# vasudeva-ram/Julia-NewtonRaphsonHANK

Measured on AMD Instinct MI355X. Metric: sequence-space JVPs/sec (household block: BackwardIteration+ForwardIteration+aggregation, Krusell-Smith T=300), higher is better.
Workload: dtype f64; 1 GPU; ks_2000x11_T300_N32; grid=2000x11, T=300, tangents_per_gpu=32, step=1 dual-sweep pass: primal + N tangents (hank_primal_jvp), parallelism=tangent-sharded x1

## Files before the change

### julia-newtonraphsonhank_amd/csrc/hank_hip.hip

```cpp
#include "hank_kernels.h"
#include "hank_xsweep.h"
#include "hank_jacobian.h"
#include "hank_wide.h"
#include "hank_hetx.h"
#include "hank_adjoint.h"
#include "hank_boundary.h"
#include "hank_ssdiff_launch.h"
#include "../../include/hank_hip.h"

#include <cstdarg>
#include <cstdio>
#include <cstdlib>
#include <cstring>
#include <initializer_list>
#include <list>
#include <mutex>
#include <new>
#include <vector>

using namespace hank;

struct FreeDevice { void operator()(void *p) const { (void)hipFree(p); } };
struct FreeGraphExec { void operator()(hipGraphExec_t g) const { (void)hipGraphExecDestroy(g); } };
template <typename H, typename Release>
// ... 702 lines not shown
    HIPC(ctx, hipMemsetAsync(X.sync, 0, sizeof(XSync) * ((size_t)2 + 2 * XPASS_MAX), ctx->stream));
    HIPC(ctx, X.st_s.alloc(2 * XG * G));
    HIPC(ctx, X.st_ds.alloc(2 * XG * G * X.dmax));
    const size_t GM = (size_t)c.n_e * X.Sact * 64;
    HIPC(ctx, X.st_D.alloc(2 * XG * std::max(GV, GM)));
    HIPC(ctx, X.st_dD.alloc(2 * XG * GM * xslots(X.dmax + 1).SP));
    HIPC(ctx, X.Dvirt.alloc(P * c.n_e * 64));
    HIPC(ctx, X.D0own.alloc(P * c.n_e));
    HIPC(ctx, X.aggpart.alloc(2 * P * (size_t)X.Sact));
    HIPC(ctx, X.rho.alloc(P));
    HIPC(ctx, X.srcB.alloc(P * X.Sact));
    HIPC(ctx, X.srcF.alloc(P * X.Sact));
    HIPC(ctx, X.unitsF.alloc(P * X.Sact * XUCAP));
    HIPC(ctx, X.unit_overflow.alloc(1));
    HIPC(ctx, hipMemsetAsync(X.unit_overflow, 0, sizeof(int), ctx->stream));
    if (const char *ng = getenv("HANK_XNEIGH")) X.neigh = atoi(ng) != 0;
    if (const char *uc = getenv("HANK_XUCAP")) X.ucap = std::min(XUCAP, std::max(1, atoi(uc)));
    {
        double ms = 20.0;
        if (const char *wm = getenv("HANK_XWAIT_MS")) ms = atof(wm);
        const unsigned long long ticks = (unsigned long long)(std::max(ms, 0.01) * 1e5);
        HIPC(ctx, hipMemcpyToSymbol(HIP_SYMBOL(hank::g_xwait_ticks), &ticks, sizeof(ticks)));
    }
    if (const char *sv = getenv("HANK_XSYNCWAVE")) X.syncwave = atoi(sv) != 0;
    X.lds_max = (int)prop.sharedMemPerBlock;
    if (const char *xf = getenv("HANK_XFAULT")) {
        X.fault = strncmp(xf, "placement", 9) == 0 ? XERR_PLACEMENT : (strncmp(xf, "timeout", 7) == 0 ? XERR_TIMEOUT : (strncmp(xf, "stall", 5) == 0 ? 3 : 0));
        const char *w = strchr(xf, ':');
        X.fault_where = !w ? 7 : (strcmp(w, ":primal") == 0 ? 1 : (strcmp(w, ":tangent") == 0 ? 2 : (strcmp(w, ":fixedpoint") == 0 ? 4 : 7)));
    }
    HIPC(ctx, hipMemsetAsync(X.Dvirt, 0, sizeof(double) * P * c.n_e * 64, ctx->stream));
    X.ready = true;
    return HANK_OK;
}

static int x_build_tan(hank_ctx *ctx, XTan &w) {
    XWork &X = ctx->xw;
    const Consts &c = ctx->c;
    const size_t P = c.P, G = c.G;
    const int N = w.N;
    size_t off = 0;
    for (int n0 = 0; n0 < N; n0 += XG * X.dmax) {
        XPass ps;
        ps.n0 = n0; ps.N = std::min(N - n0, XG * X.dmax);
        ps.D = 1; while (XG * ps.D < ps.N) ps.D *= 2;
        ps.groups = (ps.N + ps.D - 1) / ps.D;
        ps.dpol_off = off;
        off += P * ps.groups * G * ps.D;
        w.passes.push_back(ps);
    }
    if ((int)w.passes.size() > XPASS_MAX) return fail(ctx, HANK_ERR_BAD_ARG, "N=%d needs %d passes, at most %d per call", N, (int)w.passes.size(), XPASS_MAX);
    HIPC(ctx, w.dxhh.alloc((size_t)c.n_hh * P * N));
    HIPC(ctx, w.dxr.alloc(P * N)); HIPC(ctx, w.dxw.alloc(P * N)); HIPC(ctx, w.dxt.alloc(P * N));
    HIPC(ctx, w.dpol.alloc(off));
    const size_t W = (size_t)XG * X.dmax, nb = (size_t)X.Sact;
    HIPC(ctx, w.daggpart.alloc(2 * P * nb * W));
    HIPC(ctx, hipMemsetAsync(w.daggpart, 0, sizeof(double) * 2 * P * nb * W, ctx->stream));
    HIPC(ctx, w.dagg_pass.alloc(2 * P * W));
    HIPC(ctx, w.dagg_cm.alloc(2 * P * N));
    return HANK_OK;
}
static int x_ensure_tan(hank_ctx *ctx, int N, XTan **out) {
    const int nmax = 8 * ctx->xw.dmax * XPASS_MAX;
    if (N > nmax) return fail(ctx, HANK_ERR_BAD_ARG, "N=%d exceeds %d directions per call", N, nmax);
    return tan_cache_get(ctx, ctx->xw.tans, N, [ctx](XTan &w) { return x_build_tan(ctx, w); }, out);
}

static dim3 x_block(const XWork &X, const Consts &c) {
    const bool fits = 64 * (c.n_e + 1) <= X.maxt && X.syncwave;
    return dim3(fits ? 64 * (c.n_e + 1) : 64 * c.n_e);
}

template <typename F>
static void x_by_maxt(const XWork &X, F launch) { if (X.maxt == 768) launch(std::integral_constant<int, 768>()); else launch(std::integral_constant<int, 1024>()); }
#define XL(...) hipLaunchKernelGGL((__VA_ARGS__), dim3(X.grid), x_block(X, c), lds, sec.stream(), a)
static bool x_has_dual_back(const XWork &X) { return X.maxt == 768; }
static void x_launch_dual_back(XSection &sec, const XWork &X, const Consts &c, int D, const XDualBackArgs &a) {
    const size_t lds = x_lds_dual_back(c, D);
    if (!x_has_dual_back(X)) return;
    if (D == 1) XL(k_xdual_back<1, 768>);
    else if (D == 2) XL(k_xdual_back<2, 768>);
    else XL(k_xdual_back<4, 768>);
}
static void x_launch_fwd(XSection &sec, const XWork &X, const Consts &c, int D, bool val, const XSweepFwdArgs &a) {
    const size_t lds = x_lds_fwd(c, D, val || D == 0);
    x_by_maxt(X, [&](auto mt) {
        constexpr int MT = decltype(mt)::value;
        if (D == 0) XL(k_xfwd<0, true, MT>);
        else if (D == 1) { if (val) XL(k_xfwd<1, true, MT>); else XL(k_xfwd<1, false, MT>); }
        else if (D == 2) { if (val) XL(k_xfwd<2, true, MT>); else XL(k_xfwd<2, false, MT>); }
        else if (D == 4) { if constexpr (MT == 768) { if (val) XL(k_xfwd<4, true, MT>); else XL(k_xfwd<4, false, MT>); } }
    });
}
static void x_launch_primal_back(XSection &sec, const XWork &X, const Consts &c, const XBackArgs &a) { const size_t lds = x_lds_primal_back(c); x_by_maxt(X, [&](auto mt) { XL(k_xprimal_back<decltype(mt)::value>); }); }
static void x_launch_tan_back(XSection &sec, const XWork &X, const Consts &c, int D, const XTanBackArgs &a) {
    const size_t lds = x_lds_tan_back(c, D);
    x_by_maxt(X, [&](auto mt) {
        constexpr int MT = decltype(mt)::value;
        if (D == 1) XL(k_xtan_back<1, MT>);
        else if (D == 2) XL(k_xtan_back<2, MT>);
        else if (D == 4) { if constexpr (MT == 768) XL(k_xtan_back<4, MT>); }
    });
}
static void x_ensure_rng(XSection &sec) {
    hank_ctx *ctx = sec.ctx;
    XWork &X = ctx->xw;
    if (X.rng_valid) return;
    hipLaunchKernelGGL(k_xunits_fwd, dim3((unsigned)ctx->c.P, (unsigned)X.Sact), dim3(256), 0, sec.stream(), ctx->c, ctx->R, X.Sact, X.srcF, X.unitsF, X.unit_overflow, X.ucap);
    X.rng_valid = true;
}

static int ensure_seg(hank_ctx *ctx) {
    if (ctx->seg_valid) return HANK_OK;
    hipLaunchKernelGGL(k_seg_build, dim3((unsigned)(ctx->c.P * ctx->c.n_e)), dim3(256), 0, ctx->stream, ctx->c, ctx->R, ctx->c.P * ctx->c.n_e);
    HIPC(ctx, hipGetLastError());
    ctx->seg_valid = true;
    return HANK_OK;
}
static int ensure_lwg(hank_ctx *ctx) {
    if (ctx->lwg_valid) return HANK_OK;
    const XWork &X = ctx->xw;
    hipLaunchKernelGGL(k_xlwg_build, dim3((unsigned)(ctx->c.P * ctx->c.n_e)), dim3(256), 0, ctx->stream, ctx->c, ctx->R, X.Dvirt, X.D0own, X.Sact);
    HIPC(ctx, hipGetLastError());
    ctx->lwg_valid = true;
    ctx->lwg_builds++;
    return HANK_OK;
}
static int x_sync_reset(XSection &sec, XSync *base, int count, int where) {
    hank_ctx *ctx = sec.ctx;
    HIPC(ctx, hipMemsetAsync(base, 0, sizeof(XSync) * (size_t)count, sec.stream()));
    if (ctx->xw.fault && ctx->xw.fault != 3 && (ctx->xw.fault_where & where)) hipLaunchKernelGGL(k_xpoison, dim3(1), dim3(64), 0, sec.stream(), base, count, (unsigned)ctx->xw.fault);
    return HANK_OK;
}

static void x_rho(XSection &sec) {
    hank_ctx *ctx = sec.ctx;
    hipLaunchKernelGGL(k_xrho, dim3((unsigned)((ctx->c.P + 255) / 256)), dim3(256), 0, sec.stream(), ctx->d_xhh, ctx->c.n_hh, ctx->c.P, ctx->xw.rho);
}
static void x_tan_in(XSection &sec, XTan *w) {
    const Consts &c = sec.ctx->c;
    hipLaunchKernelGGL(k_tan_in, dim3((unsigned)(((size_t)c.P * w->N + 255) / 256)), dim3(256), 0, sec.stream(), w->dxhh, c.n_hh, c.P, w->N, w->dxr, w->dxw, w->dxt);
}
static int x_tan_front(XSection &sec, XTan *w) {
    hank_ctx *ctx = sec.ctx; XWork &X = ctx->xw;
    const int rc = x_sync_reset(sec, X.sync + 2, 2 * (int)w->passes.size(), 2); if (rc) return rc;
    x_tan_in(sec, w);
    x_rho(sec);
    if (!X.src_valid) {
        hipLaunchKernelGGL(k_xsrc_back, dim3((unsigned)ctx->c.P, X.Sact), dim3(256), 0, sec.stream(), ctx->c, ctx->R, X.Sact, X.srcB);
        X.src_valid = true;
    }
    return HANK_OK;
}
static int x_back(XSection &sec, XTan *dual = nullptr) {
    hank_ctx *ctx = sec.ctx; XWork &X = ctx->xw;
    const Consts &c = ctx->c;
    XBackArgs ab{};
    ab.c = c; ab.ss_value = ctx->d_ss_value; ab.xhh = ctx->d_xhh; ab.rho = X.rho; ab.sy = X.sync; ab.st_s = X.st_s;
    ab.err = ctx->d_err; ab.R = ctx->R;
    HIPC(ctx, ctx->spans.begin(PRIMAL_BACK, sec.stream()));
    if (dual) {
        const XPass &ps = dual->passes[0];
        XDualBackArgs db{};
        db.p = ab; db.dxr = dual->dxr; db.dxw = dual->dxw; db.dxt = dual->dxt; db.Ntot = dual->N; db.n0 = ps.n0; db.N = ps.N;
        db.st_ds = X.st_ds; db.dpol = dual->dpol + ps.dpol_off; db.groups = ps.groups;
        x_launch_dual_back(sec, X, c, ps.D, db);
    } else x_launch_primal_back(sec, X, c, ab);
    HIPC(ctx, ctx->spans.end(PRIMAL_BACK, sec.stream(), 1));
    return HANK_OK;
}
static void x_lottery(XSection &sec, bool seg) {
    hank_ctx *ctx = sec.ctx;
    const Consts &c = ctx->c;
    hipLaunchKernelGGL(k_lottery, dim3((unsigned)(c.P * c.n_e)), dim3(256), sizeof(int) * (2 * (size_t)c.n_a + 2), sec.stream(), c, ctx->R, c.P * c.n_e, ctx->d_err, seg ? 1 : 0, 1);
}
static int x_tan_back(XSection &sec, XTan *w) {
    hank_ctx *ctx = sec.ctx; XWork &X = ctx->xw;
    const int np = (int)w->passes.size();
    XTanBackArgs ab{};
    ab.c = ctx->c; ab.R = ctx->R; ab.rho = X.rho; ab.xhh = ctx->d_xhh; ab.dxr = w->dxr; ab.dxw = w->dxw; ab.dxt = w->dxt; ab.Ntot = w->N; ab.st_ds = X.st_ds;
    ab.src = X.neigh ? X.srcB.get() : nullptr;
    ab.stall = X.fault == 3 ? 1 : 0;
    HIPC(ctx, ctx->spans.begin(TAN_BACK, sec.stream()));
    for (int p = 0; p < np; p++) {
        const XPass &ps = w->passes[p];
        ab.n0 = ps.n0; ab.N = ps.N; ab.groups = ps.groups; ab.sy = X.sync + 2 + 2 * p; ab.dpol = w->dpol + ps.dpol_off;
        x_launch_tan_back(sec, X, ctx->c, ps.D, ab);
    }
    HIPC(ctx, ctx->spans.end(TAN_BACK, sec.stream(), np));
    return HANK_OK;
}
static void x_value_epilogue(XSection &sec) {
    hank_ctx *ctx = sec.ctx; const XWork &X = ctx->xw;
    const Consts &c = ctx->c;
    const size_t P = c.P;
    hipStream_t s = sec.stream();
    hipLaunchKernelGGL(k_reduce_parts, dim3((unsigned)P, 1), dim3(256), 0, s, X.aggpart, X.Sact, 2, ctx->d_agg_rm);
    hipLaunchKernelGGL(k_tan_out, dim3((unsigned)((2 * P + 255) / 256)), dim3(256), 0, s, ctx->d_agg_rm, (int)P, 2, ctx->d_agg);
    hipLaunchKernelGGL(k_xfix_D, dim3((unsigned)((P * c.n_e + 255) / 256)), dim3(256), 0, s, c, ctx->R.Dseq, X.Dvirt, X.Sact, X.D0own);
}
static XSweepFwdArgs x_fwd_args(const hank_ctx *ctx, bool val) {
    const XWork &X = ctx->xw;
    XSweepFwdArgs fa{};
    fa.c = ctx->c; fa.R = ctx->R; fa.src = X.srcF; fa.units = X.unitsF; fa.overflow = X.unit_overflow; fa.all_members = X.neigh ? 0 : 1;
    if (val) { fa.D0 = ctx->d_ss_D; fa.Dvirt = X.Dvirt; fa.aggpart = X.aggpart; }
    return fa;
}
static int x_fwd_value(XSection &sec) {
    hank_ctx *ctx = sec.ctx; XWork &X = ctx->xw;
    XSweepFwdArgs fa = x_fwd_args(ctx, true);
    fa.sy = X.sync + 1; fa.st = X.st_D; fa.groups = 1;
    HIPC(ctx, ctx->spans.begin(PRIMAL_FWD, sec.stream()));
    x_launch_fwd(sec, X, ctx->c, 0, true, fa);
    HIPC(ctx, ctx->spans.end(PRIMAL_FWD, sec.stream(), 1));
    x_value_epilogue(sec);
    return HANK_OK;
}
static int x_tan_fwd(XSection &sec, XTan *w, int p, bool val) {
    hank_ctx *ctx = sec.ctx; XWork &X = ctx->xw;
    const XPass &ps = w->passes[p];
    if (!val) { const int rc = ensure_lwg(ctx); if (rc) return rc; }
    XSweepFwdArgs fa = x_fwd_args(ctx, val);
    fa.sy = X.sync + 2 + 2 * p + 1; fa.st = X.st_dD; fa.daggpart = w->daggpart; fa.groups = ps.groups; fa.dpol = w->dpol + ps.dpol_off;
    x_launch_fwd(sec, X, ctx->c, ps.D, val, fa);
    return HANK_OK;
}
static void x_tan_reduce(XSection &sec, XTan *w, int p) {
    hank_ctx *ctx = sec.ctx;
    const size_t P = ctx->c.P;
    const XPass &ps = w->passes[p];
    const int W = XG * ps.D;
    hipStream_t s = sec.stream();
    hipLaunchKernelGGL(k_reduce_parts, dim3((unsigned)P, (2 * W + 63) / 64), dim3(256), 0, s, w->daggpart, ctx->xw.Sact, 2 * W, w->dagg_pass);
    hipLaunchKernelGGL(k_xout, dim3((unsigned)((P * ps.N + 255) / 256)), dim3(256), 0, s, w->dagg_pass, (int)P, 2 * W, 0, ps.n0, ps.N, w->dagg_cm);
    hipLaunchKernelGGL(k_xout, dim3((unsigned)((P * ps.N + 255) / 256)), dim3(256), 0, s, w->dagg_pass, (int)P, 2 * W, W, ps.n0, ps.N, w->dagg_cm + P * (size_t)w->N);
}
static int x_tan_fwd_from(XSection &sec, XTan *w, int first) {
    hank_ctx *ctx = sec.ctx;
    const int np = (int)w->passes.size();
    for (int p = first; p < np; p++) {
        const int rc = x_tan_fwd(sec, w, p, false); if (rc) return rc;
        if (p == np - 1) HIPC(ctx, ctx->spans.end(TAN_FWD, sec.stream(), np));
        x_tan_reduce(sec, w, p);
    }
    return HANK_OK;
}
static void x_dual_epilogue(XSection &sec, XTan *w, double *d_agg_out, double *d_dagg_out) {
    hank_ctx *ctx = sec.ctx; const XWork &X = ctx->xw;
    const Consts &c = ctx->c;
    const XPass &ps = w->passes[0];
    const int W = XG * ps.D, per = 2 * W + 2 + c.n_e;
    hipLaunchKernelGGL(k_xdual_epilogue, dim3((unsigned)(((size_t)c.P * per + 255) / 256)), dim3(256), 0, sec.stream(), c, X.aggpart, w->daggpart, X.Sact, W, ps.n0, ps.N, w->N,
                       ctx->d_agg_rm, ctx->d_agg, w->dagg_pass, w->dagg_cm, ctx->R.Dseq, X.Dvirt, X.D0own, d_agg_out, d_dagg_out);
}

static int x_status(hank_ctx *ctx, const char *what, const XSync *fetched) {
    XWork &X = ctx->xw;
    std::vector<XSync> own;
    if (!fetched) {
        if (!X.ready || X.last_blocks == 0) return HANK_OK;
        int uo = 0;
        HIPC(ctx, hipMemcpy(&uo, X.unit_overflow, sizeof(int), hipMemcpyDeviceToHost));
        if (uo) {
            HIPC(ctx, hipMemsetAsync(X.unit_overflow, 0, sizeof(int), ctx->stream));
            return fail(ctx, HANK_ERR_SWEEP, "persistent forward sweep: a member's walk over its sources needs more than %d work units (a savings policy this flat is served by the per-period launches)", XUCAP);
        }
        own.resize((size_t)X.last_blocks);
        HIPC(ctx, hipMemcpy(own.data(), X.sync, sizeof(XSync) * own.size(), hipMemcpyDeviceToHost));
    }
    const XSync *h = fetched ? fetched : own.data();
    for (size_t k = 0; k < (fetched ? 1 : own.size()); k++)
        if (h[k].status[0] != 0) {
            if (what) return fail(ctx, HANK_ERR_SWEEP, "persistent %s: %s on XCD %u", what, h[k].status[0] == XERR_PLACEMENT ? "the group is short of members" : "a wait timed out", h[k].status[1]);
            char waited[64] = "";
            if (h[k].status[0] == XERR_TIMEOUT) snprintf(waited, sizeof(waited), " after %.1f ms", h[k].status[2] / 1000.0);
            return fail(ctx, HANK_ERR_SWEEP, "persistent %s sweep %zu (0 = primal, then one per tangent pass): %s%s on XCD %u (workgroups per XCD: %u %u %u %u %u %u %u %u)",
                        (k & 1) ? "forward" : "backward", k / 2, h[k].status[0] == XERR_PLACEMENT ? "a group is short of members" : "a wait timed out", waited,
                        h[k].status[1], h[k].ticket[0][0], h[k].ticket[1][0], h[k].ticket[2][0], h[k].ticket[3][0], h[k].ticket[4][0],
                        h[k].ticket[5][0], h[k].ticket[6][0], h[k].ticket[7][0]);
        }
    return HANK_OK;
}

#define HANK_WIDE_NE_LIST(X) X(2) X(3) X(4) X(5) X(7) X(11)
static bool w_ne_instantiated(int ne) {
#define X(NEV) if (ne == NEV) return true;
    HANK_WIDE_NE_LIST(X)
#undef X
    return false;
}
struct WGeom { int R, maxt, kreg_b, kreg_f; };
static WGeom w_geom(const hank_ctx *ctx) { return ctx->wide_r == 2 ? WGeom{2, 1024, 16, 7} : WGeom{4, 512, 16, 16}; }
static int w_threads(const hank_ctx *ctx) { const WGeom g = w_geom(ctx); return std::max(64, ((ctx->c.n_a + g.R - 1) / g.R + 63) / 64 * 64); }
static size_t w_lds(const hank_ctx *ctx) { const WGeom g = w_geom(ctx); return std::max(wide_lds_back(ctx->c, g.kreg_b), wide_lds_fwd(ctx->c, g.kreg_f)); }
static bool w_supported(const hank_ctx *ctx) {
    const Consts &c = ctx->c;
    return w_ne_instantiated(c.n_e) && c.n_a <= WIDE_CS && w_lds(ctx) <= ctx->lds_max &&
           ctx->rec_bytes < 0x7fffffffull && (size_t)c.G * sizeof(double) < 0x7fffffffull;
}
static bool use_wide(const hank_ctx *ctx, int N) {
    if (ctx->wide_mode == 2) return true;
    if (ctx->wide_mode != 1) return false;
    const int rounds = (N + ctx->num_cus - 1) / ctx->num_cus;
    return (long long)N * 256 >= (long long)rounds * ctx->wide_min * ctx->num_cus;
}

template <int NE, int R, int MAXT, int KB, int KF>
static int w_launch_geom(XSection &sec, bool fwd, int N, const WideArgs &a) {
    hank_ctx *ctx = sec.ctx;
    const Consts &c = ctx->c;
    WMat<NE> M;
    for (int k = 0; k < NE; k++)
        for (int e = 0; e < NE; e++) M.m[k * NE + e] = fwd ? ctx->h_Pi[k + NE * e] : ctx->h_Pi[e + NE * k];
    for (int e = 0; e < NE; e++) M.z[e] = ctx->h_z[e];
    const dim3 grd((unsigned)N), blk((unsigned)w_threads(ctx));
    if (fwd) {
        const size_t lds = wide_lds_fwd(c, KF);
        HIPC(ctx, hipFuncSetAttribute(reinterpret_cast<const void *>(&k_wide_fwd<NE, R, MAXT, KF>), hipFuncAttributeMaxDynamicSharedMemorySize, (int)lds));
        hipLaunchKernelGGL((k_wide_fwd<NE, R, MAXT, KF>), grd, blk, lds, sec.stream(), a, M);
    } else {
        const size_t lds = wide_lds_back(c, KB);
        if (c.diet) {
            HIPC(ctx, hipFuncSetAttribute(reinterpret_cast<const void *>(&k_wide_back<NE, R, MAXT, true, KB>), hipFuncAttributeMaxDynamicSharedMemorySize, (int)lds));
            hipLaunchKernelGGL((k_wide_back<NE, R, MAXT, true, KB>), grd, blk, lds, sec.stream(), a, M);
        } else {
            HIPC(ctx, hipFuncSetAttribute(reinterpret_cast<const void *>(&k_wide_back<NE, R, MAXT, false, KB>), hipFuncAttributeMaxDynamicSharedMemorySize, (int)lds));
            hipLaunchKernelGGL((k_wide_back<NE, R, MAXT, false, KB>), grd, blk, lds, sec.stream(), a, M);
        }
    }
    return HANK_OK;
}
static int w_launch(XSection &sec, bool fwd, int N, const WideArgs &a) {
    hank_ctx *ctx = sec.ctx;
#define X(NEV) if (ctx->c.n_e == NEV) return ctx->wide_r == 2 ? w_launch_geom<NEV, 2, 1024, 16, 7>(sec, fwd, N, a) : w_launch_geom<NEV, 4, 512, 16, 16>(sec, fwd, N, a);
    HANK_WIDE_NE_LIST(X)
#undef X
    return fail(ctx, HANK_ERR_BAD_ARG, "on-chip wide sweeps: n_e=%d is not instantiated", ctx->c.n_e);
}

static int w_ensure_tan(hank_ctx *ctx, int N, bool staging, WTan **out) {
    const size_t P = ctx->c.P, G = ctx->c.G;
    const int rc = tan_cache_get(ctx, ctx->wtans, N, [=](WTan &w) -> int {
        HIPC(ctx, w.dpol.alloc(P * (size_t)N * G + 2));
        HIPC(ctx, w.dagg_cm.alloc(2 * P * (size_t)N));
        return HANK_OK;
    }, out);
    if (rc) return rc;
    if (staging && !(*out)->dxhh) HIPC(ctx, (*out)->dxhh.alloc((size_t)ctx->c.n_hh * P * N));
    return HANK_OK;
}

static int w_run_tangent(hank_ctx *ctx, WTan *w, const double *d_dxhh) {
    const Consts &c = ctx->c;
    XSection sec(ctx);
    HIPC(ctx, sec.opened());
    hipStream_t s = sec.stream();
    if (!ctx->d_ibw) HIPC(ctx, ctx->d_ibw.alloc((size_t)c.P * c.G + 4));
    WideArgs a{};
    a.c = c; a.R = ctx->R; a.xhh = ctx->d_xhh; a.dxhh = d_dxhh; a.Ntot = w->N; a.n0 = 0; a.dpol = w->dpol; a.dagg = w->dagg_cm;
    a.rec = ctx->rec_slab;
    auto off = [&](const void *p) { return (unsigned)((const char *)p - ctx->rec_slab); };
    const Record &R = ctx->R;
    a.o_s = off(R.s); a.o_kc = off(R.kc); a.o_u = off(R.u); a.o_v = off(R.v); a.ibw = ctx->d_ibw;
    a.nrank = std::max(1, std::min(ctx->num_cus / 8, w->N / 8));
    a.o_lwg = off(R.lwg); a.o_start = off(R.start); a.o_D = off(R.Dseq); a.o_pol = off(R.pol);
    if (!ctx->wprep_valid) {
        const size_t npt = (size_t)c.P * c.G;
        hipLaunchKernelGGL(k_wide_prep, dim3((unsigned)((npt + 255) / 256)), dim3(256), 0, s, R.ib, R.A, R.B, npt, ctx->d_ibw);
        ctx->wprep_valid = true;
    }
    HIPC(ctx, ctx->spans.begin(TAN_BACK, s));
    int rc = w_launch(sec, false, w->N, a);
    if (rc) return rc;
    HIPC(ctx, ctx->spans.end(TAN_BACK, s, 1));
    HIPC(ctx, join_side(ctx));
    rc = ensure_lwg(ctx);
// ... 258 lines not shown
    HIPC(ctx, hipEventRecord(ctx->ev_fork, ctx->stream));
    HIPC(ctx, hipStreamWaitEvent(ctx->side_stream, ctx->ev_fork, 0));
    HIPC(ctx, ctx->spans.begin(PRIMAL_FWD, ctx->side_stream));
    HIPC(ctx, hipGraphLaunch(ctx->g_pfwd, ctx->side_stream));
    HIPC(ctx, ctx->spans.end(PRIMAL_FWD, ctx->side_stream, ctx->c.P + 1));
    HIPC(ctx, copy_agg(ctx, d_agg_out, hipMemcpyDeviceToDevice, ctx->side_stream));
    HIPC(ctx, hipEventRecord(ctx->ev_side, ctx->side_stream));
    ctx->side_pending = true;
    ctx->spans.invalidate({DUAL_BACK, DUAL_FWD});
    record_rewritten(ctx, true, true);
    return HANK_OK;
}

static int x_primal(hank_ctx *ctx, const double *xhh, hipMemcpyKind kind, double *d_agg_out) {
    int rc = x_setup(ctx); if (rc) return rc;
    HIPC(ctx, hipMemcpyAsync(ctx->d_xhh, xhh, sizeof(double) * ctx->c.n_hh * ctx->c.P, kind, ctx->stream));
    XSection sec(ctx);
    HIPC(ctx, sec.opened());
    rc = x_sync_reset(sec, ctx->xw.sync, 2, 1); if (rc) return rc;
    zero_err(ctx, sec.stream());
    x_rho(sec);
    rc = x_back(sec); if (rc) return rc;
    x_lottery(sec, true);
    record_rewritten(ctx, true, HANK_XPRIMAL_LWG_IN_SWEEP);
    x_ensure_rng(sec);
    rc = x_fwd_value(sec); if (rc) return rc;
    HIPC(ctx, hipGetLastError());
    HIPC(ctx, sec.close());
    ctx->stats[SWEEP_LAUNCHES] += 2;
    ctx->xw.last_blocks = 2;
    ctx->spans.invalidate({TAN_BACK, TAN_FWD, DUAL_BACK, DUAL_FWD});
    HIPC(ctx, copy_agg(ctx, d_agg_out, hipMemcpyDeviceToDevice, ctx->stream));
    return HANK_OK;
}
static int x_jvp(hank_ctx *ctx, const double *dxhh, hipMemcpyKind kind, int N, double *d_dagg_out) {
    int rc = x_setup(ctx); if (rc) return rc;
    XTan *w = nullptr;
    rc = x_ensure_tan(ctx, N, &w); if (rc) return rc;
    const int np = (int)w->passes.size();
    HIPC(ctx, hipMemcpyAsync(w->dxhh, dxhh, sizeof(double) * ctx->c.n_hh * ctx->c.P * N, kind, ctx->stream));
    XSection sec(ctx);
    HIPC(ctx, sec.opened());
    rc = x_tan_front(sec, w); if (rc) return rc;
    x_ensure_rng(sec);
    rc = x_tan_back(sec, w); if (rc) return rc;
    HIPC(ctx, ctx->spans.begin(TAN_FWD, sec.stream()));
    rc = x_tan_fwd_from(sec, w, 0); if (rc) return rc;
    HIPC(ctx, hipGetLastError());
    HIPC(ctx, sec.close());
    ctx->stats[SWEEP_LAUNCHES] += 2 * np;
    ctx->xw.last_blocks = 2 + 2 * np;
    ctx->spans.invalidate({DUAL_BACK, DUAL_FWD});
    batch_ran(ctx, 1, w, N, w->dagg_cm, w->dpol, &w->passes);
    HIPC(ctx, copy_dagg(ctx, d_dagg_out, w->dagg_cm, N, hipMemcpyDeviceToDevice));
    return HANK_OK;
}
static void x_dual_ran(hank_ctx *ctx, XTan *w, int launches) {
    ctx->stats[SWEEP_LAUNCHES] += launches;
    ctx->xw.last_blocks = 2 + 2 * (int)w->passes.size();
    ctx->spans.absent(PRIMAL_FWD, 1);
    ctx->spans.invalidate({DUAL_BACK, DUAL_FWD});
    batch_ran(ctx, 1, w, w->N, w->dagg_cm, w->dpol, &w->passes);
}
static int x_dual_two(hank_ctx *ctx, XTan *w, const double *xhh, const double *dxhh, hipMemcpyKind kind, double *d_agg_out, double *d_dagg_out) {
    const size_t nP = (size_t)ctx->c.n_hh * ctx->c.P;
    const int np = (int)w->passes.size();
    XSection sec(ctx);
    HIPC(ctx, sec.opened());
    HIPC(ctx, hipMemcpyAsync(w->dxhh, dxhh, sizeof(double) * nP * w->N, kind, sec.stream()));
    HIPC(ctx, hipMemcpyAsync(ctx->d_xhh, xhh, sizeof(double) * nP, kind, sec.stream()));
    int rc = x_sync_reset(sec, ctx->xw.sync, 2, 1); if (rc) return rc;
    zero_err(ctx, sec.stream());
    x_rho(sec);
    rc = x_back(sec); if (rc) return rc;
    x_lottery(sec, true);
    record_rewritten(ctx, true, false);
    x_ensure_rng(sec);
    rc = x_tan_front(sec, w);
    if (!rc) rc = x_tan_back(sec, w);
    if (rc) return rc;
    HIPC(ctx, ctx->spans.begin(TAN_FWD, sec.stream()));
    rc = x_tan_fwd(sec, w, 0, true); if (rc) return rc;
    if (np == 1) {
        HIPC(ctx, ctx->spans.end(TAN_FWD, sec.stream(), 1));
        x_dual_epilogue(sec, w, d_agg_out, d_dagg_out);
    } else {
        x_value_epilogue(sec);
        x_tan_reduce(sec, w, 0);
        rc = x_tan_fwd_from(sec, w, 1); if (rc) return rc;
    }
    HIPC(ctx, hipGetLastError());
    HIPC(ctx, sec.close());
    x_dual_ran(ctx, w, 1 + 2 * np);
    if (np > 1) {
        HIPC(ctx, copy_agg(ctx, d_agg_out, hipMemcpyDeviceToDevice, ctx->stream));
        HIPC(ctx, copy_dagg(ctx, d_dagg_out, w->dagg_cm, w->N, hipMemcpyDeviceToDevice));
    }
    return HANK_OK;
}
static int x_dual_fused(hank_ctx *ctx, XTan *w, const double *xhh, const double *dxhh, hipMemcpyKind kind, bool prologue, double *d_agg_out, double *d_dagg_out) {
    XWork &X = ctx->xw;
    const size_t nP = (size_t)ctx->c.n_hh * ctx->c.P;
    XSection sec(ctx);
    HIPC(ctx, sec.opened());
    if (prologue) {
        hipLaunchKernelGGL(k_xdual_prologue, dim3(64), dim3(256), 0, sec.stream(), xhh, ctx->d_xhh, dxhh, w->dxhh, ctx->c.n_hh, ctx->c.P, w->N, X.rho, w->dxr, w->dxw, w->dxt,
                           reinterpret_cast<xv4u *>(X.sync.get()), sizeof(XSync) * 4 / sizeof(xv4u), ctx->d_err);
    } else {
        HIPC(ctx, hipMemcpyAsync(w->dxhh, dxhh, sizeof(double) * nP * w->N, kind, sec.stream()));
        HIPC(ctx, hipMemcpyAsync(ctx->d_xhh, xhh, sizeof(double) * nP, kind, sec.stream()));
        int rc = x_sync_reset(sec, X.sync, 2, 1);
        if (!rc) rc = x_sync_reset(sec, X.sync + 2, 2, 2);
        if (rc) return rc;
        zero_err(ctx, sec.stream());
        x_rho(sec);
        x_tan_in(sec, w);
    }
    int rc = x_back(sec, w); if (rc) return rc;
    x_lottery(sec, false);
    record_rewritten(ctx, false, false);
    x_ensure_rng(sec);
    HIPC(ctx, ctx->spans.begin(TAN_BACK, sec.stream()));
    HIPC(ctx, ctx->spans.end(TAN_BACK, sec.stream(), 1));
    HIPC(ctx, ctx->spans.begin(TAN_FWD, sec.stream()));
    rc = x_tan_fwd(sec, w, 0, true); if (rc) return rc;
    HIPC(ctx, ctx->spans.end(TAN_FWD, sec.stream(), 1));
    x_dual_epilogue(sec, w, d_agg_out, d_dagg_out);
    HIPC(ctx, hipGetLastError());
    HIPC(ctx, sec.close());
    x_dual_ran(ctx, w, 2);
    return HANK_OK;
}
static bool x_dual_back_fits(const hank_ctx *ctx, int D);
static int x_dual(hank_ctx *ctx, const double *xhh, const double *dxhh, hipMemcpyKind kind, int N, double *d_agg_out, double *d_dagg_out) {
    int rc = x_setup(ctx); if (rc) return rc;
    XTan *w = nullptr;
    rc = x_ensure_tan(ctx, N, &w); if (rc) return rc;
    if (w->passes.size() != 1 || !x_dual_back_fits(ctx, w->passes[0].D)) return x_dual_two(ctx, w, xhh, dxhh, kind, d_agg_out, d_dagg_out);
    return x_dual_fused(ctx, w, xhh, dxhh, kind, kind == hipMemcpyDeviceToDevice && !ctx->xw.fault, d_agg_out, d_dagg_out);
}
static bool use_x_primal(const hank_ctx *ctx) { return ctx->schedule >= 1; }
static bool x_tan_fits(const hank_ctx *ctx, int N) {
    const XWork &X = ctx->xw;
    int D = 1;
    while (XG * D < N && D < X.dmax) D *= 2;
    return std::max(x_lds_tan_back(ctx->c, D), x_lds_fwd(ctx->c, D, true)) <= (size_t)X.lds_max;
}
static bool use_x_jvp(const hank_ctx *ctx, int N) { return (ctx->schedule == 1 || (ctx->schedule == 2 && N <= ctx->xjvp_max)) && x_tan_fits(ctx, N); }
static bool x_dual_back_fits(const hank_ctx *ctx, int D) {
    const XWork &X = ctx->xw;
    return ctx->xdual_back && x_has_dual_back(X) && 64 * (ctx->c.n_e + 1) <= X.maxt && x_lds_dual_back(ctx->c, D) <= (size_t)X.lds_max;
}
static bool use_x_fused(const hank_ctx *ctx, int N) {
    if (ctx->schedule < 1 || !x_tan_fits(ctx, N)) return false;
    if (ctx->schedule == 1) return true;
    return N <= XG * ctx->xw.dmax && x_dual_back_fits(ctx, ctx->xw.dmax);
}

static int check_rates(hank_ctx *ctx, const double *xhh) {
    for (int t = 0; t < ctx->c.P; t++)
        if (!(1.0 + xhh[ctx->c.n_hh * t] > 0.0)) return fail(ctx, HANK_ERR_DOMAIN, "1 + r must be positive (period %zu)", (size_t)t + 1);
    return HANK_OK;
}
static int enqueue_primal(hank_ctx *ctx, const double *xhh, hipMemcpyKind kind, double *d_agg_out) {
    if (use_x_primal(ctx)) return x_primal(ctx, xhh, kind, d_agg_out);
    HIPC(ctx, hipMemcpyAsync(ctx->d_xhh, xhh, sizeof(double) * ctx->c.n_hh * ctx->c.P, kind, ctx->stream));
    return run_primal(ctx, d_agg_out);
}

int hank_primal_dev(hank_ctx *ctx, const double *d_xhh, double *d_agg_out) {
    ENTER(ctx);
    if (!ctx || !d_xhh) return fail(ctx, HANK_ERR_BAD_ARG, "null pointer");
    if (!ctx->boundary_set) return fail(ctx, HANK_ERR_NOT_READY, "hank_set_boundary must be called first");
    note_primal_x(ctx, nullptr);
    ctx->stats[PRIMAL_SWEEPS]++;
    return enqueue_primal(ctx, d_xhh, hipMemcpyDeviceToDevice, d_agg_out);
}

int hank_check(hank_ctx *ctx) {
    ENTER(ctx);
    if (!ctx) return HANK_ERR_BAD_ARG;
    bool moved = false;
    return fallback_decision(ctx, device_verdict(ctx, THE_RECORD), &moved);
}

int hank_primal(hank_ctx *ctx, const double *xhh, double *agg_out) {
    ENTER(ctx);
    if (!ctx || !xhh) return fail(ctx, HANK_ERR_BAD_ARG, "null pointer");
    if (!ctx->boundary_set) return fail(ctx, HANK_ERR_NOT_READY, "hank_set_boundary must be called first");
    { const int rrc = check_rates(ctx, xhh); if (rrc) return rrc; }
    note_primal_x(ctx, nullptr);
    const int rc = run_settled(ctx, [&] { return enqueue_primal(ctx, xhh, hipMemcpyHostToDevice, nullptr); });
    if (rc) return rc;
    if (agg_out) {
        HIPC(ctx, copy_agg(ctx, agg_out, hipMemcpyDeviceToHost, ctx->stream));
        HIPC(ctx, hipStreamSynchronize(ctx->stream));
    }
    note_primal_x(ctx, xhh);
    ctx->stats[PRIMAL_SWEEPS]++;
    ctx->errmsg[0] = 0;
    return HANK_OK;
}

static int run_jvp(hank_ctx *ctx, TanWork &w, bool bnd, bool zm, int NX) {
    const int grc = ensure_tan_graphs(ctx, w, bnd, NX);
    if (grc) return grc;
    HIPC(ctx, ctx->spans.begin(TAN_BACK, ctx->stream));
    HIPC(ctx, hipGraphLaunch(w.tan_back(bnd), ctx->stream));
    HIPC(ctx, ctx->spans.end(TAN_BACK, ctx->stream, ctx->c.P + (bnd ? 4 : 2)));
    HIPC(ctx, join_side(ctx));
    { const int src = ensure_seg(ctx); if (src) return src; }
    { const int src = ensure_lwg(ctx); if (src) return src; }
    HIPC(ctx, ctx->spans.begin(TAN_FWD, ctx->stream));
    HIPC(ctx, hipGraphLaunch(w.tan_fwd(bnd, NX), ctx->stream));
    HIPC(ctx, ctx->spans.end(TAN_FWD, ctx->stream, ctx->c.P + (bnd ? 5 : 3) + (NX > 0 ? 1 : 0)));
    if (bnd) batch_ran_boundary(ctx, &w, w.N, w.dagg_cm, w.dpol, zm ? w.bnd_zm.get() : nullptr);
    else batch_ran(ctx, 0, &w, w.N, w.dagg_cm, w.dpol);
    return HANK_OK;
}

struct TanReq {
    int n_het;
    const double *dxhh, *dvalue_end, *dD_init;
    hipMemcpyKind kind;
    bool seeded;
};
static int ensure_bnd_bufs(hank_ctx *ctx, TanWork &w);
static int ensure_hx_record(hank_ctx *ctx);

static int enqueue_tan_launch(hank_ctx *ctx, const TanReq &q, int N, TanWork **out) {
    const Consts &c = ctx->c;
    const size_t P = c.P, GN = (size_t)c.G * N;
    const int NX = q.n_het > 2 ? q.n_het - 2 : 0, SX = hx_count(ctx);
    TanWork *w = nullptr;
    int rc = ensure_tanwork(ctx, N, &w);
    if (rc) return rc;
    if (q.seeded && (rc = ensure_bnd_bufs(ctx, *w)) != HANK_OK) return rc;
    if (q.n_het > 0 && !w->het_out) HIPC(ctx, w->het_out.alloc(P * het_max(ctx) * N));
    if (NX > 0) {
        HIPC(ctx, join_side(ctx));
        rc = ensure_hx_record(ctx);
        if (rc) return rc;
        if (!w->hx_T) {
            HIPC(ctx, w->hx_parts.alloc(P * (size_t)w->nbf * SX * N));
            HIPC(ctx, w->hx_T.alloc((size_t)N * P * SX));
        }
    }
    const struct { double *dst; const double *src; size_t count; } in[3] = {{w->dxhh, q.dxhh, c.n_hh * P * N}, {w->bnd_dV, q.dvalue_end, GN}, {w->bnd_dD, q.dD_init, GN}};
    for (int k = 0; k < (q.seeded ? 3 : 1); k++) {
        if (in[k].src) HIPC(ctx, hipMemcpyAsync(in[k].dst, in[k].src, sizeof(double) * in[k].count, q.kind, ctx->stream));
        else HIPC(ctx, hipMemsetAsync(in[k].dst, 0, sizeof(double) * in[k].count, ctx->stream));
    }
    rc = run_jvp(ctx, *w, q.seeded, q.dD_init != nullptr, NX);
    if (rc) return rc;
    *out = w;
    return HANK_OK;
}
static int enqueue_tan_raw(hank_ctx *ctx, const TanReq &q, int N, double *d_dagg_out) {
    TanWork *w = nullptr;
    const int rc = enqueue_tan_launch(ctx, q, N, &w);
    if (rc) return rc;
    HIPC(ctx, copy_dagg(ctx, d_dagg_out, w->dagg_cm, N, hipMemcpyDeviceToDevice));
    return HANK_OK;
}
static int tan_host_tail(hank_ctx *ctx, double *out, const double *d_src, size_t count) {
    HIPC(ctx, hipMemcpyAsync(out, d_src, sizeof(double) * count, hipMemcpyDeviceToHost, ctx->stream));
    HIPC(ctx, hipStreamSynchronize(ctx->stream));
    ctx->errmsg[0] = 0;
    return HANK_OK;
}
static int tan_seed_args(hank_ctx *ctx, const char *who, bool het, const TanReq &q, int N, const void *out, bool need_out) {
    if (!ctx || (!q.dxhh && !q.dvalue_end && !q.dD_init) || (need_out && !out) || N < 1)
        return fail(ctx, HANK_ERR_BAD_ARG, "%s: bad argument (N=%d; at least one of dxhh, dvalue_end, dD_init must be given)", who, N);
    const int rc = het ? het_count_ok(ctx, who, q.n_het, true) : HANK_OK;
    if (rc) return rc;
    if (!ctx->primal_done) return fail(ctx, HANK_ERR_NOT_READY, "hank_primal must be called before %s", who);
    return HANK_OK;
}

static int enqueue_jvp(hank_ctx *ctx, const double *dxhh, hipMemcpyKind kind, int N, double *d_dagg_out) {
    if (use_wide(ctx, N)) return w_jvp(ctx, dxhh, kind, N, d_dagg_out);
    if (use_x_jvp(ctx, N)) return x_jvp(ctx, dxhh, kind, N, d_dagg_out);
    return enqueue_tan_raw(ctx, TanReq{0, dxhh, nullptr, nullptr, kind, false}, N, d_dagg_out);
}

int hank_jvp_dev(hank_ctx *ctx, const double *d_dxhh, int32_t N, double *d_dagg_out) {
    ENTER(ctx);
    if (!ctx || !d_dxhh || N < 1) return fail(ctx, HANK_ERR_BAD_ARG, "bad argument (N=%d)", N);
    if (!ctx->primal_done) return fail(ctx, HANK_ERR_NOT_READY, "hank_primal must be called before hank_jvp");
    return enqueue_jvp(ctx, d_dxhh, hipMemcpyDeviceToDevice, N, d_dagg_out);
}

int hank_jvp(hank_ctx *ctx, const double *dxhh, int32_t N, double *dagg_out) {
    ENTER(ctx);
    if (!ctx || !dxhh || !dagg_out || N < 1) return fail(ctx, HANK_ERR_BAD_ARG, "bad argument (N=%d)", N);
    if (!ctx->primal_done) return fail(ctx, HANK_ERR_NOT_READY, "hank_primal must be called before hank_jvp");
    int rc = enqueue_jvp(ctx, dxhh, hipMemcpyHostToDevice, N, nullptr);
    if (rc) return rc;
    if (ctx->batch.family == 2) rc = device_verdict(ctx, THE_RECORD);
    else if (ctx->batch.family == 1) {
        bool rerun = false;
        rc = settle(ctx, &rerun);
        if (rerun) {
            rc = run_primal(ctx, nullptr);
            if (!rc) rc = device_verdict(ctx, THE_RECORD);
            if (!rc) rc = enqueue_jvp(ctx, dxhh, hipMemcpyHostToDevice, N, nullptr);
        }
// ... 1306 lines not shown
```

### julia-newtonraphsonhank_amd/csrc/hank_kernels.h

```cpp
#pragma once
#include <hip/hip_runtime.h>
#include <stdint.h>

namespace hank {

constexpr int RBP = 32;

struct Consts {
    int n_a, n_e, G, P;
    int n_hh;
    int diet;
    double beta, gamma, bc;
    const double *a, *z, *Pi;
};

struct Record {
    double *s, *kc, *A, *B, *u, *v, *pol, *lw, *ig, *Dseq;
    int *ib, *lo, *start, *clo;
    int4 *seg;
    double2 *lwg;
};

enum { ERR_KNOTS = 3, ERR_DOMAIN = 4, ERR_NONMONO = 6 };

__device__ inline void set_err(int *err, int code, int t, int e, int j) {
    if (atomicCAS(&err[0], 0, code) == 0) {
        err[1] = t;
        err[2] = e;
        err[3] = j;
    }
}

__device__ inline bool pow_domain_error(double v, double y) { return (v < 0.0) && (y != floor(y)); }

#ifndef HANK_IEEE_DIV
#define HANK_IEEE_DIV 0
#endif
__device__ __forceinline__ double fast_rcp(double x) {
#if HANK_IEEE_DIV
    return 1.0 / x;
#else
    double r = __builtin_amdgcn_rcp(x);
    r = __builtin_fma(__builtin_fma(-x, r, 1.0), r, r);
    r = __builtin_fma(__builtin_fma(-x, r, 1.0), r, r);
    return r;
#endif
}
__device__ __forceinline__ double fast_rsqrt(double x) {
#if HANK_IEEE_DIV
    return 1.0 / sqrt(x);
#else
    double y = __builtin_amdgcn_rsq(x);
    y = __builtin_fma(y * 0.5, __builtin_fma(-(x * y), y, 1.0), y);
    y = __builtin_fma(y * 0.5, __builtin_fma(-(x * y), y, 1.0), y);
    return y;
#endif
}
__device__ __forceinline__ double fast_sqrt(double x) {
#if HANK_IEEE_DIV
    return sqrt(x);
#else
    const double y = fast_rsqrt(x), g = x * y;
    return __builtin_fma(y * 0.5, __builtin_fma(-g, g, x), g);
#endif
}

__device__ inline double pow_crra(double x, double y) {
    if (y == -0.5) return fast_rsqrt(x);
    if (y == -2.0) return fast_rcp(x * x);
    if (y == -1.0) return fast_rcp(x);
    return pow(x, y);
}

__device__ inline double wave_sum(double x) {
#pragma unroll
    for (int off = 32; off > 0; off >>= 1) x += __shfl_down(x, off, 64);
    return x;
}
__device__ inline double block_sum(double x, double *red, int nthreads) {
    const int lane = threadIdx.x & 63, wv = threadIdx.x >> 6;
    const int nw = (nthreads + 63) >> 6;
    x = wave_sum(x);
    __syncthreads();
    if (lane == 0) red[wv] = x;
    __syncthreads();
    double r = 0.0;
    if (threadIdx.x == 0)
        for (int k = 0; k < nw; k++) r += red[k];
    return r;
}

#ifndef HANK_RAW_BARRIER
#define HANK_RAW_BARRIER 1
#endif
__device__ __forceinline__ void lds_barrier() {
#if HANK_RAW_BARRIER
    asm volatile("s_waitcnt lgkmcnt(0)\n\ts_barrier" ::: "memory");
#else
    __syncthreads();
#endif
}

#ifndef HANK_ST_DPOL
#define HANK_ST_DPOL 1
#endif
#ifndef HANK_ST_STATE
#define HANK_ST_STATE 1
#endif
#ifndef HANK_ST_REC
#define HANK_ST_REC 0
#endif
template <int MODE>
__device__ __forceinline__ void st_mode(double *p, double x) {
    if (MODE == 1) __hip_atomic_store(reinterpret_cast<unsigned long long *>(p), (unsigned long long)__double_as_longlong(x), __ATOMIC_RELAXED, __HIP_MEMORY_SCOPE_AGENT);
    else if (MODE == 2) __builtin_nontemporal_store(x, p);
    else *p = x;
}
template <int MODE>
__device__ __forceinline__ void st_mode_i(int *p, int x) {
    if (MODE == 1) __hip_atomic_store(p, x, __ATOMIC_RELAXED, __HIP_MEMORY_SCOPE_AGENT);
    else if (MODE == 2) __builtin_nontemporal_store(x, p);
    else *p = x;
}

__device__ __forceinline__ double mix_mul(double p, double v) { return p * v; }
__device__ __forceinline__ double2 mix_mul(double p, double2 v) { return make_double2(p * v.x, p * v.y); }
__device__ __forceinline__ double mix_add(double a, double b) { return a + b; }
__device__ __forceinline__ double2 mix_add(double2 a, double2 b) { return make_double2(a.x + b.x, a.y + b.y); }
template <typename T>
__device__ __forceinline__ T mix_sum(T acc, const T *V, int vs, const double *P, int ps, int k0, int n) {
    int k = k0;
    for (; k + 3 < n; k += 4) {
        const T v0 = V[k * vs], v1 = V[(k + 1) * vs], v2 = V[(k + 2) * vs], v3 = V[(k + 3) * vs];
        const double p0 = P[k * ps], p1 = P[(k + 1) * ps], p2 = P[(k + 2) * ps], p3 = P[(k + 3) * ps];
        acc = mix_add(acc, mix_mul(p0, v0));
        acc = mix_add(acc, mix_mul(p1, v1));
        acc = mix_add(acc, mix_mul(p2, v2));
        acc = mix_add(acc, mix_mul(p3, v3));
    }
    if (k + 1 < n) {
        const T v0 = V[k * vs], v1 = V[(k + 1) * vs];
        const double p0 = P[k * ps], p1 = P[(k + 1) * ps];
        acc = mix_add(acc, mix_mul(p0, v0));
        acc = mix_add(acc, mix_mul(p1, v1));
        k += 2;
    }
    if (k < n) acc = mix_add(acc, mix_mul(P[k * ps], V[k * vs]));
    return acc;
}

__device__ __forceinline__ double diet_kc(const Consts &c, double s, double rho, double opr, double wz_tr, double xa) {
    const double cm = (s * opr + wz_tr) - xa;
    const double k = rho * (c.beta * (-1.0 / c.gamma));
    return c.gamma == 2.0 ? k * (cm * cm * cm) : k * (cm * cm);
}
__device__ __forceinline__ double diet_v(const Consts &c, double u, double opr) {
    return c.gamma == 2.0 ? opr * (-2.0 * (u * fast_sqrt(u))) : opr * (-(u * u));
}

__device__ __forceinline__ double hh_tr(const Consts &c, const double *xhh, int t) { return c.n_hh > 2 ? xhh[c.n_hh * t + 2] : 0.0; }

__device__ inline void egm_X(const Consts &c, const double *Vsh, const double *Pish, int row, int a,
                             int e, double r, double w, double tr, double *s_out, double *kc_out, int *err,
                             int t) {
    const double E = mix_sum(Vsh[row] * Pish[e], Vsh + row, RBP, Pish + e, c.n_e, 1, c.n_e);
    const double bE = E * c.beta;
    const double ex = -1.0 / c.gamma;
    if (pow_domain_error(bE, ex)) set_err(err, ERR_DOMAIN, t, e, a);
    const double cm = pow_crra(bE, ex);
    const double rho = 1.0 / (1.0 + r);
    const double s1 = rho * ((cm - (w * c.z[e] + tr)) + c.a[a]);
    st_mode<HANK_ST_REC>(s_out, s1);
    st_mode<HANK_ST_REC>(kc_out, c.diet ? diet_kc(c, s1, rho, 1.0 + r, w * c.z[e] + tr, c.a[a]) : rho * (c.beta * ex * (cm / bE)));
}

struct YOut {
    double g, A, B, u, v, V;
    int ib;
};
enum { Y_INSIDE = 0, Y_BELOW = 1, Y_ABOVE = 2 };
struct YFront {
    int where, i;
    double si, sj;
    bool slow;
    bool bad;
};
template <typename KNOTS> struct YFrontOf { static constexpr bool value = false; };
template <typename KNOTS> struct YColumnZOf { static constexpr bool value = false; };
constexpr int Y_WAIT_VMCNT0 = 0x0F70;

template <bool ZREG>
__device__ __forceinline__ YOut egm_Y_finish(const Consts &c, int a, int e, double r, double w, double tr, int *err, int t,
                                             double x, double g, double A, double B, int i, double ze) {
    YOut o;
    const double bc = c.bc;
    if ((bc > g) || ((int)signbit(bc) < (int)signbit(g))) {
        A = 0.0;
        B = 0.0;
    }
    g = (g > bc) ? g : ((bc > g) ? bc : (signbit(g) ? bc : g));
    const double opr = 1.0 + r;
    const double cg = (opr * x + (w * (ZREG ? ze : c.z[e]) + tr)) - g;
    if (pow_domain_error(cg, -c.gamma)) set_err(err, ERR_DOMAIN, t, e, a);
    const double u = pow_crra(cg, -c.gamma);
    o.g = g;
    o.A = A;
    o.B = B;
    o.ib = i;
    o.u = u;
    o.v = c.diet ? diet_v(c, u, opr) : opr * ((-c.gamma) * (u / cg));
    o.V = opr * u;
    return o;
}

template <typename KNOTS>
__device__ inline YOut egm_Y(const Consts &c, const KNOTS sc, int a, int e, double r, double w, double tr,
                             int *err, int t, int guess) {
    constexpr bool FRONT = YFrontOf<KNOTS>::value;
    const int n = c.n_a;
    const double x = c.a[a];
    double s0, sN, si, sj;
    int where, i;
    bool slow, slow_wave;
    if constexpr (FRONT) {
        const YFront f = sc.front(x, guess);
        where = f.where; i = f.i; si = f.si; sj = f.sj;
        slow = f.slow;
        slow_wave = __any(f.slow || f.bad) != 0;
        if (slow_wave) {
            if (f.bad) set_err(err, ERR_KNOTS, t, e, a);
        }
    } else {
        const double sa = sc[a];
        if (a > 0 ? !(sa > sc[a - 1]) : !(sa == sa)) set_err(err, ERR_KNOTS, t, e, a);
        s0 = sc[0]; sN = sc[n - 1];
    }
    double g, A = 0.0, B = 0.0;
    if (FRONT ? where == Y_BELOW : x < s0) {
        g = c.a[0];
        i = 0;
    } else if (FRONT ? where == Y_ABOVE : x > sN) {
        g = c.a[n - 1];
        i = n - 2;
    } else {
        if (FRONT ? slow_wave : true) {
            if (FRONT ? slow : true) {
                int lo = -1, hi = n;
                bool have = false;
                double vlo = 0.0, vhi = 0.0;
                if (guess >= 0) {
                    const int p = guess < n - 1 ? guess : n - 2;
                    const int pm = p > 0 ? p - 1 : 0, pp = p + 2 < n ? p + 2 : n - 1;
                    const double sm = sc[pm], sp = sc[p], sp1 = sc[p + 1], sp2 = sc[pp];
                    if (sp <= x && x < sp1) {
                        lo = p; hi = p + 1; have = true; vlo = sp; vhi = sp1;
                    } else if (p + 2 < n && sp1 <= x && x < sp2) {
                        lo = p + 1; hi = p + 2; have = true; vlo = sp1; vhi = sp2;
                    } else if (p > 0 && sm <= x && x < sp) {
                        lo = p - 1; hi = p; have = true; vlo = sm; vhi = sp;
                    } else if (sp1 <= x) {
                        lo = p + 1;
                        for (int step = 1;; step <<= 1) {
                            const int q = lo + step;
                            if (q >= n) break;
                            if (sc[q] <= x) lo = q; else { hi = q; break; }
                        }
                    } else {
                        hi = p;
                        for (int step = 1;; step <<= 1) {
                            const int q = hi - step;
                            if (q < 0) break;
                            if (sc[q] <= x) { lo = q; break; } else hi = q;
                        }
                    }
                }
                while (hi - lo > 1) {
// ... 861 lines not shown
```

### julia-newtonraphsonhank_amd/csrc/hank_wide.h

```cpp
#pragma once
#include "hank_xsweep.h"

namespace hank {

constexpr int WIDE_CS = 2048;
constexpr int wide_kl(int ne, int kreg) { return ne > kreg ? ne - kreg : 0; }
template <int NE> struct WMat { double m[NE * NE]; double z[NE]; };

__device__ __forceinline__ double wide_uniform(double v) {
    return __hiloint2double(__builtin_amdgcn_readfirstlane(__double2hiint(v)), __builtin_amdgcn_readfirstlane(__double2loint(v)));
}
__device__ __forceinline__ void wide_pin(double &v) { asm volatile("" : "+v"(v)); }
__device__ __forceinline__ int wide_opaque_zero(int t, int q) { return __builtin_amdgcn_readfirstlane((t >> (27 + (q & 3))) & 1); }

template <int NE, int R, int KR, int LSTRIDE>
__device__ __forceinline__ void wide_mix(double (&x)[R][KR], double *lst, const double *m, int zero) {
#pragma clang fp contract(fast)
    constexpr int KL = NE - KR;
    double y[R][NE], cf[2][NE], xl[2][R];
    int off = zero;
#pragma unroll
    for (int e = 0; e < NE; e++) cf[0][e] = m[off + e];
#pragma unroll
    for (int k = 0; k < NE; k++) {
        if (k + 1 < NE) {
            if (k == 0) asm volatile("" : "+s"(off) : "v"(x[0][0]));
            else asm volatile("" : "+s"(off) : "v"(y[R - 1][NE - 1]));
#pragma unroll
            for (int e = 0; e < NE; e++) cf[(k + 1) & 1][e] = m[off + (k + 1) * NE + e];
            if (k + 1 >= KR) {
#pragma unroll
                for (int q = 0; q < R; q++) xl[(k + 1) & 1][q] = lst[((k + 1 - KR) * R + q) * LSTRIDE];
            }
        }
        if (k == 0 && KR == 0) {
#pragma unroll
            for (int q = 0; q < R; q++) xl[0][q] = lst[q * LSTRIDE];
        }
#pragma unroll
        for (int q = 0; q < R; q++) {
            const double xk = k < KR ? x[q][k < KR ? k : 0] : xl[k & 1][q];
#pragma unroll
            for (int e = 0; e < NE; e++) { y[q][e] = k == 0 ? cf[0][e] * xk : y[q][e] + cf[k & 1][e] * xk; asm volatile("" : "+v"(y[q][e])); }
        }
        __builtin_amdgcn_sched_barrier(0);
    }
#pragma unroll
    for (int q = 0; q < R; q++) {
#pragma unroll
        for (int e = 0; e < KR; e++) { x[q][e] = y[q][e]; asm volatile("" : "+v"(x[q][e])); }
#pragma unroll
        for (int k = 0; k < KL; k++) lst[(k * R + q) * LSTRIDE] = y[q][KR + k];
    }
    __builtin_amdgcn_sched_barrier(0);
}

typedef unsigned int wv2u __attribute__((ext_vector_type(2)));
typedef unsigned int wv4u __attribute__((ext_vector_type(4)));
__device__ __forceinline__ __amdgpu_buffer_rsrc_t wide_rsrc(const void *p) {
    return __builtin_amdgcn_make_buffer_rsrc(const_cast<void *>(p), 0, 0x7fffffff, 0x00020000);
}
__device__ __forceinline__ double wide_ld64(__amdgpu_buffer_rsrc_t rs, int vo, int so) {
    const wv2u q = __builtin_amdgcn_raw_buffer_load_b64(rs, vo, so, 0);
    return __hiloint2double((int)q.y, (int)q.x);
}
__device__ __forceinline__ wv2u wide_ld2i(__amdgpu_buffer_rsrc_t rs, int vo, int so) { return __builtin_amdgcn_raw_buffer_load_b64(rs, vo, so, 0); }
template <int AUX>
__device__ __forceinline__ void wide_ld2d(__amdgpu_buffer_rsrc_t rs, int vo, int so, double &a, double &b) {
    const wv4u q = __builtin_amdgcn_raw_buffer_load_b128(rs, vo, so, AUX);
    a = __hiloint2double((int)q.y, (int)q.x); b = __hiloint2double((int)q.w, (int)q.z);
}
__device__ __forceinline__ wv4u wide_ld128(__amdgpu_buffer_rsrc_t rs, int vo, int so) { return __builtin_amdgcn_raw_buffer_load_b128(rs, vo, so, 0); }
__device__ __forceinline__ void wide_st2d_nt(double a, double b, __amdgpu_buffer_rsrc_t rs, int vo, int so) {
    wv4u q;
    q.x = (unsigned)__double2loint(a); q.y = (unsigned)__double2hiint(a); q.z = (unsigned)__double2loint(b); q.w = (unsigned)__double2hiint(b);
    __builtin_amdgcn_raw_buffer_store_b128(q, rs, vo, so, 2);
}
__device__ __forceinline__ void wide_st64_nt(double v, __amdgpu_buffer_rsrc_t rs, int vo, int so) {
    wv2u q;
    q.x = (unsigned)__double2loint(v); q.y = (unsigned)__double2hiint(v);
    __builtin_amdgcn_raw_buffer_store_b64(q, rs, vo, so, 2);
}

#ifdef HANK_WIDE_TIMING_L2
#define WIDE_TPER(t) ((t) & 1)
#else
#define WIDE_TPER(t) (t)
#endif
#ifdef HANK_XSTAMP
__device__ unsigned long long g_wstamps[2][4][64];
#define WSTAMP(sw, per, i)                                                                                          \
    do {                                                                                                            \
        if (blockIdx.x == 0 && threadIdx.x == 0 && (per) >= 100 && (per) < 104) g_wstamps[sw][(per) - 100][i] = __builtin_amdgcn_s_memtime(); \
    } while (0)
#else
#define WSTAMP(sw, per, i) do {} while (0)
#endif

struct WideArgs {
    Consts c;
    Record R;
    const double *xhh;
    const double *dxhh;
    int Ntot, n0;
    double *dpol;
    double *dagg;
    const void *rec;
    unsigned o_s, o_kc, o_u, o_v, o_lwg, o_start, o_D, o_pol;
    const int *ibw;
    int nrank;
};

static inline size_t wide_lds_back(const Consts &c, int kreg) {
    return sizeof(double) * (4 * (size_t)WIDE_CS + (size_t)WIDE_CS + 8 * (size_t)c.P + (size_t)wide_kl(c.n_e, kreg) * WIDE_CS);
}
static inline size_t wide_lds_fwd(const Consts &c, int kreg) {
    return sizeof(double) * (4 * (size_t)WIDE_CS + 96 + (size_t)WIDE_CS + (size_t)wide_kl(c.n_e, kreg) * WIDE_CS) + sizeof(int) * ((size_t)c.P * c.n_e + 4);
}

template <int R>
struct WideRows {
    int row[R], o8[R / 2], o4[R / 2], o16[R / 2];
    bool ok[R];
    __device__ __forceinline__ void init(int NT, int tid, int na) {
#pragma unroll
        for (int j = 0; j < R / 2; j++) {
            const int r0 = 2 * (j * NT + tid);
            row[2 * j] = r0; row[2 * j + 1] = r0 + 1;
            ok[2 * j] = r0 < na; ok[2 * j + 1] = r0 + 1 < na;
            const int rc = ok[2 * j] ? r0 : 0;
            o8[j] = rc * 8; o4[j] = rc * 4; o16[j] = rc * 16;
        }
    }
};

template <int NE, int R, int MAXT, bool DIET, int KREG>
__global__ void __launch_bounds__(MAXT) k_wide_back(WideArgs A, WMat<NE> M) {
#pragma clang fp contract(fast)
    static_assert(R % 2 == 0 && R * MAXT == WIDE_CS, "rows come in adjacent pairs; a workgroup covers WIDE_CS rows");
    constexpr int KL = wide_kl(NE, KREG), KR = NE - KL, CS = R * MAXT;
    extern __shared__ __attribute__((aligned(16))) double xl[];
    const Consts &c = A.c;
    const int na = c.n_a, P = c.P, NT = blockDim.x, tid = threadIdx.x, G = c.G;
    const int n = A.n0 + blockIdx.x;
    double2 *buf = reinterpret_cast<double2 *>(xl);
    double *dash = xl + 4 * (size_t)CS;
    double *uni = dash + CS;
    double *lst = uni + 8 * (size_t)P + tid;
    for (int k = tid; k < P; k += NT) {
        const double r = A.xhh[c.n_hh * k];
        const double *dx = A.dxhh + (size_t)c.n_hh * ((size_t)k + (size_t)P * n);
        uni[8 * k] = 1.0 / (1.0 + r); uni[8 * k + 1] = 1.0 + r; uni[8 * k + 2] = A.xhh[c.n_hh * k + 1]; uni[8 * k + 3] = hh_tr(c, A.xhh, k);
        uni[8 * k + 4] = dx[0]; uni[8 * k + 5] = dx[1]; uni[8 * k + 6] = c.n_hh > 2 ? dx[2] : 0.0; uni[8 * k + 7] = 0.0;
    }
    for (int k = tid; k < CS; k += NT) dash[k] = k + 1 < na ? c.a[k + 1] - c.a[k] : 1.0;
    WideRows<R> rw;
    rw.init(NT, tid, na);
    double xa[R];
#pragma unroll
    for (int q = 0; q < R; q++) xa[q] = c.a[rw.ok[q] ? rw.row[q] : 0];
    double dV[R][KR];
#pragma unroll
    for (int q = 0; q < R; q++) {
#pragma unroll
        for (int e = 0; e < KR; e++) dV[q][e] = 0.0;
#pragma unroll
        for (int k = 0; k < KL; k++) lst[(k * R + q) * MAXT] = 0.0;
    }
    const __amdgpu_buffer_rsrc_t rs = wide_rsrc(A.rec), rs_w = wide_rsrc(A.ibw);
    struct Stage { double s[R], kc[DIET ? 1 : R], cu[R], cv[R]; int ib[R]; } S;
    auto load_X = [&](int so) {
#pragma unroll
        for (int j = 0; j < R / 2; j++) {
            wide_ld2d<0>(rs, rw.o8[j], A.o_s + so * 8, S.s[2 * j], S.s[2 * j + 1]);
            if constexpr (!DIET) wide_ld2d<0>(rs, rw.o8[j], A.o_kc + so * 8, S.kc[2 * j], S.kc[2 * j + 1]);
        }
    };
    auto load_Y1 = [&](int so) {
#pragma unroll
        for (int j = 0; j < R / 2; j++) {
            const wv2u iq = wide_ld2i(rs_w, rw.o4[j], so * 4);
            S.ib[2 * j] = (int)iq.x; S.ib[2 * j + 1] = (int)iq.y;
        }
    };
    auto load_Y2 = [&](int so) {
#pragma unroll
        for (int j = 0; j < R / 2; j++) {
            wide_ld2d<0>(rs, rw.o8[j], A.o_u + so * 8, S.cu[2 * j], S.cu[2 * j + 1]);
            wide_ld2d<0>(rs, rw.o8[j], A.o_v + so * 8, S.cv[2 * j], S.cv[2 * j + 1]);
        }
    };
    const int tch_line = ((int)(blockIdx.x >> 3) % A.nrank + A.nrank * tid) * 128;
    const int tch_n8 = G * 8, tch_n4 = G * 4;
    constexpr int TCH_ARR = DIET ? 3 : 4;
    int tch_arr = 0, tch_off = tch_line;
#pragma unroll
    for (int k = 1; k < TCH_ARR; k++)
        if (tch_off >= tch_n8) { tch_off -= tch_n8; tch_arr = k; }
    const int tch_v8 = tch_off < tch_n8 ? (int)(tch_arr == 0 ? A.o_s : tch_arr == 1 ? A.o_u : tch_arr == 2 ? A.o_v : A.o_kc) + tch_off : (int)0x80000000;
    const int tch_v4 = tch_line < tch_n4 ? tch_line : (int)0x80000000;
    unsigned tch_j8 = 0, tch_j4 = 0;
    __syncthreads();
    { const int so = WIDE_TPER(P - 1) * G; load_X(so); load_Y1(so); load_Y2(so); }
    int pb = 0;
    for (int t = P - 1; t >= 0; t--) {
        WSTAMP(0, t, 0);
#ifndef HANK_WIDE_NO_TOUCH
        asm volatile("" :: "v"(tch_j8), "v"(tch_j4));
        {
            const int tb = WIDE_TPER(t > 0 ? t - 1 : 0) * G;
            tch_j8 = __builtin_amdgcn_raw_buffer_load_b32(rs, tch_v8, tb * 8, 0);
            tch_j4 = __builtin_amdgcn_raw_buffer_load_b32(rs_w, tch_v4, tb * 4, 0);
        }
#endif
        const double rho = wide_uniform(uni[8 * t]), opr = wide_uniform(uni[8 * t + 1]), w = wide_uniform(uni[8 * t + 2]), tr = wide_uniform(uni[8 * t + 3]);
        const double dr = wide_uniform(uni[8 * t + 4]), dw = wide_uniform(uni[8 * t + 5]), dtr = wide_uniform(uni[8 * t + 6]);
        wide_mix<NE, R, KR, MAXT>(dV, lst, M.m, wide_opaque_zero(t, 1));
        const int zt = wide_opaque_zero(t, 0);
        const __amdgpu_buffer_rsrc_t rs_dp = wide_rsrc(A.dpol + ((size_t)t * A.Ntot + n) * (size_t)G);
        WSTAMP(0, t, 1);
#pragma unroll
        for (int e = 0; e < NE; e++) {
            const int last = e + 1 == NE;
            const int son = WIDE_TPER(last ? (t > 0 ? t - 1 : 0) : t) * G + (last ? 0 : e + 1) * na + zt;
            const double ze = M.z[e], wz = w * ze + tr, zd = ze * dw + dtr;
            double2 *const col = buf + pb * CS;
            double ds[R];
#pragma unroll
            for (int q = 0; q < R; q++) {
                const double dE = e < KR ? dV[q][e < KR ? e : 0] : lst[((e - KR) * R + q) * MAXT];
                double kc;
                if constexpr (DIET) kc = diet_kc(c, S.s[q], rho, opr, wz, xa[q]); else kc = S.kc[q];
                ds[q] = kc * dE - rho * (zd + S.s[q] * dr);
                wide_pin(ds[q]);
            }
// ... 233 lines not shown
```

### julia-newtonraphsonhank_amd/csrc/hank_xsweep.h

```cpp
#pragma once
#ifndef HANK_XFWD_PRECOMBINE
#define HANK_XFWD_PRECOMBINE 1
#endif
#ifndef HANK_XBACK_FRONT
#define HANK_XBACK_FRONT 1
#endif
#ifndef HANK_XBACK_ZREG
#define HANK_XBACK_ZREG 1
#endif
#include "hank_kernels.h"
#include <type_traits>

namespace hank {

constexpr int XG = 8;
constexpr int XRW = 63;
enum { XERR_TIMEOUT = 1, XERR_PLACEMENT = 2 };
__device__ unsigned long long g_xwait_ticks = 2000000ull;
struct XDeadline {
    unsigned long long t0;
    __device__ __forceinline__ XDeadline() : t0(__builtin_amdgcn_s_memrealtime()) {}
    __device__ __forceinline__ bool expired(unsigned spins) const { return (spins & 63u) == 63u && __builtin_amdgcn_s_memrealtime() - t0 > g_xwait_ticks; }
    __device__ __forceinline__ unsigned waited_us() const { return (unsigned)((__builtin_amdgcn_s_memrealtime() - t0) / 100ull); }
};

struct XSync {
    unsigned ticket[XG][32];
    unsigned total[32];
    unsigned flag[XG][64][32];
    unsigned status[32];
    unsigned pad[32];
};
constexpr size_t XCTL_BYTES = 64;

typedef unsigned int xv4u __attribute__((ext_vector_type(4)));

__device__ __forceinline__ double xld(const double *p) {
    return __longlong_as_double((long long)__hip_atomic_load(reinterpret_cast<const unsigned long long *>(p), __ATOMIC_RELAXED, __HIP_MEMORY_SCOPE_AGENT));
}
__device__ __forceinline__ unsigned xldu(const unsigned *p) { return __hip_atomic_load(p, __ATOMIC_RELAXED, __HIP_MEMORY_SCOPE_AGENT); }

template <int D>
struct XRows {
    __amdgpu_buffer_rsrc_t rs;
    double *base;
    size_t plane;
    __device__ __forceinline__ void init(double *p, size_t rows_total) {
        base = p; plane = rows_total;
        if (D >= 2) rs = __builtin_amdgcn_make_buffer_rsrc(p, 0, (int)(rows_total * 8 * D), 0x00020000);
    }
    __device__ __forceinline__ void load(size_t row, double *v) const {
        if (D == 1) {
            v[0] = xld(base + row);
        } else {
#pragma unroll
            for (int k = 0; k < D / 2; k++) {
                const xv4u q = __builtin_amdgcn_raw_buffer_load_b128(rs, (int)((k * plane + row) * 16), 0, 16);
                v[2 * k] = __hiloint2double((int)q.y, (int)q.x);
                v[2 * k + 1] = __hiloint2double((int)q.w, (int)q.z);
            }
        }
    }
    __device__ __forceinline__ double load_one(size_t row, int k) const {
        return D == 1 ? xld(base + row) : xld(base + ((size_t)(k / 2) * plane + row) * 2 + (k & 1));
    }
    __device__ __forceinline__ void store(size_t row, const double *v) const {
        if (D == 1) {
            base[row] = v[0];
        } else {
#pragma unroll
            for (int k = 0; k < D / 2; k++) reinterpret_cast<double2 *>(base)[k * plane + row] = make_double2(v[2 * k], v[2 * k + 1]);
        }
    }
};
typedef double xv2d __attribute__((ext_vector_type(2)));
template <int D>
__device__ __forceinline__ void xstore_row(double *p, const double *v) {
    if (D == 1) {
        __builtin_nontemporal_store(v[0], p);
    } else {
#pragma unroll
        for (int k = 0; k < D / 2; k++) { xv2d q; q.x = v[2 * k]; q.y = v[2 * k + 1]; __builtin_nontemporal_store(q, reinterpret_cast<xv2d *>(p) + k); }
    }
}
template <int D>
__device__ __forceinline__ void xload_row_plain(const double *p, double *v) {
    if (D == 1) {
        v[0] = *p;
    } else {
#pragma unroll
        for (int k = 0; k < D / 2; k++) { const double2 q = reinterpret_cast<const double2 *>(p)[k]; v[2 * k] = q.x; v[2 * k + 1] = q.y; }
    }
}

struct XGroup { int x, c, S, ok; };

#ifdef HANK_XSTAMP
#ifndef HANK_XSTAMP_T0
#define HANK_XSTAMP_T0 100
#endif
#ifndef HANK_XSTAMP_STRIDE
#define HANK_XSTAMP_STRIDE 1
#endif
constexpr int XSTAMP_T0 = HANK_XSTAMP_T0, XSTAMP_NP = 8, XSTAMP_NS = 12, XSTAMP_ST = HANK_XSTAMP_STRIDE;
#define XSTAMP_ON(per) ((per) >= XSTAMP_T0 && (per) < XSTAMP_T0 + XSTAMP_NP * XSTAMP_ST && ((per) - XSTAMP_T0) % XSTAMP_ST == 0)
#define XSTAMP_SLOT(per) (((per) - XSTAMP_T0) / XSTAMP_ST)
__device__ unsigned long long g_xstamps[2][32][XSTAMP_NP][XSTAMP_NS];
#define XSTAMP(sw, on, per, i)                                                                                   \
    do {                                                                                                         \
        if ((on) >= 0 && XSTAMP_ON(per) && threadIdx.x == 0)                 \
            g_xstamps[sw][on][XSTAMP_SLOT(per)][i] = __builtin_amdgcn_s_memrealtime();                              \
    } while (0)
#define XSTAMPW(sw, on, per, i, wave)                                                                            \
    do {                                                                                                         \
        if ((on) >= 0 && XSTAMP_ON(per) && (int)threadIdx.x == 64 * (wave))  \
            g_xstamps[sw][on][XSTAMP_SLOT(per)][i] = __builtin_amdgcn_s_memrealtime();                              \
    } while (0)
__device__ unsigned long long g_xwaves[2][32][XSTAMP_NP][16];
#define XSTAMPV(sw, on, per)                                                                                     \
    do {                                                                                                         \
        if ((on) >= 0 && XSTAMP_ON(per) && (threadIdx.x & 63) == 0)          \
            g_xwaves[sw][on][XSTAMP_SLOT(per)][threadIdx.x >> 6] = __builtin_amdgcn_s_memrealtime();             \
    } while (0)
#define XSTAMP1(sw, on, i) do { if ((on) >= 0 && threadIdx.x == 0) g_xstamps[sw][on][0][i] = __builtin_amdgcn_s_memrealtime(); } while (0)
#else
#define XSTAMP1(sw, on, i) do {} while (0)
#define XSTAMPV(sw, on, per) do {} while (0)
#define XSTAMP(sw, on, per, i) do {} while (0)
#define XSTAMPW(sw, on, per, i, wave) do {} while (0)
#endif

__device__ inline void xfail(XSync *sy, unsigned code, int x, unsigned waited_us = 0u) {
    if (__hip_atomic_exchange(&sy->status[0], code, __ATOMIC_RELAXED, __HIP_MEMORY_SCOPE_AGENT) == 0u) {
        __hip_atomic_store(&sy->status[1], (unsigned)x, __ATOMIC_RELAXED, __HIP_MEMORY_SCOPE_AGENT);
        __hip_atomic_store(&sy->status[2], waited_us, __ATOMIC_RELAXED, __HIP_MEMORY_SCOPE_AGENT);
    }
}

__global__ void k_xpoison(XSync *base, int count, unsigned code) {
    if ((int)threadIdx.x < count) { base[threadIdx.x].status[0] = code; base[threadIdx.x].status[1] = 0u; }
}

__device__ inline XGroup xgroup_join(XSync *sy, int *ctl) {
    if (threadIdx.x == 0) {
        int xcc;
        asm volatile("s_getreg_b32 %0, hwreg(HW_REG_XCC_ID)" : "=s"(xcc));
        xcc &= 7;
        if (xldu(&sy->status[0]) != 0u) {
            ctl[0] = xcc; ctl[1] = 0; ctl[2] = 0; ctl[3] = 0;
        } else {
            const unsigned c = __hip_atomic_fetch_add(&sy->ticket[xcc][0], 1u, __ATOMIC_RELAXED, __HIP_MEMORY_SCOPE_AGENT);
            asm volatile("s_waitcnt vmcnt(0)" ::: "memory");
            __hip_atomic_fetch_add(&sy->total[0], 1u, __ATOMIC_RELAXED, __HIP_MEMORY_SCOPE_AGENT);
            int ok = 1;
            const XDeadline dl;
            for (unsigned spins = 0;; spins++) {
                if (xldu(&sy->total[0]) >= gridDim.x) break;
                if (dl.expired(spins) || ((spins & 255u) == 255u && xldu(&sy->status[0]) != 0u)) { xfail(sy, XERR_TIMEOUT, xcc, dl.waited_us()); ok = 0; break; }
                __builtin_amdgcn_s_sleep(2);
            }
            ctl[0] = xcc; ctl[1] = (int)c; ctl[2] = (int)xldu(&sy->ticket[xcc][0]); ctl[3] = ok;
        }
    }
    __syncthreads();
    XGroup g;
    g.x = __builtin_amdgcn_readfirstlane(ctl[0]); g.c = __builtin_amdgcn_readfirstlane(ctl[1]);
    g.S = __builtin_amdgcn_readfirstlane(ctl[2]); g.ok = __builtin_amdgcn_readfirstlane(ctl[3]);
    return g;
}

__device__ __forceinline__ void xlds_barrier() { asm volatile("s_waitcnt lgkmcnt(0)\n\ts_barrier" ::: "memory"); }

__device__ __forceinline__ void xbar_arrive(bool drain) {
    if (drain) asm volatile("s_waitcnt vmcnt(0)" ::: "memory");
    xlds_barrier();
}
__device__ __forceinline__ void xbar_wait(XSync *sy, int x, int c, int members, unsigned episode, bool sync_wave) {
    if (sync_wave) {
        const int lane = threadIdx.x & 63;
        if (lane == 0) *reinterpret_cast<volatile unsigned *>(&sy->flag[x][c][0]) = episode;
        const XDeadline dl;
        for (unsigned spins = 0;; spins++) {
            const unsigned f = lane < members ? xldu(&sy->flag[x][lane][0]) : episode;
            if (__all((int)(f - episode) >= 0)) break;
            if (dl.expired(spins) || ((spins & 255u) == 255u && xldu(&sy->status[0]) != 0u)) {
                if (lane == 0) xfail(sy, XERR_TIMEOUT, x, dl.waited_us());
                break;
            }
            __builtin_amdgcn_s_sleep(1);
        }
    }
    xlds_barrier();
}

__device__ __forceinline__ void xpoll(XSync *sy, int x, int lo, int hi, unsigned need) {
    const int lane = threadIdx.x & 63;
    const XDeadline dl;
    for (unsigned spins = 0;; spins++) {
        const unsigned f = (lane >= lo && lane <= hi) ? xldu(&sy->flag[x][lane][0]) : need;
        if (__all((int)(f - need) >= 0)) break;
        if (dl.expired(spins) || ((spins & 255u) == 255u && xldu(&sy->status[0]) != 0u)) {
            if (lane == 0) xfail(sy, XERR_TIMEOUT, x, dl.waited_us());
            break;
        }
        __builtin_amdgcn_s_sleep(1);
    }
}
__device__ __forceinline__ void xpublish(XSync *sy, int x, int c, unsigned episode) {
    if ((threadIdx.x & 63) == 0) *reinterpret_cast<volatile unsigned *>(&sy->flag[x][c][0]) = episode;
}

struct XKnots {
    const double *p;
    int a, n, i0, i1, i2, i3;
    double sa, sam1, s0, sN, w0, w1, w2, w3;
    double ze;
    __device__ __forceinline__ void preload(const double *col, int a_, int n_, int guess, double ze_) {
        p = col; a = a_; n = n_; ze = ze_;
        sa = xld(col + a);
        sam1 = xld(col + (a > 0 ? a - 1 : 0));
        s0 = xld(col);
        sN = xld(col + n - 1);
        i0 = i1 = i2 = i3 = -1;
        w0 = w1 = w2 = w3 = 0.0;
        if (guess >= 0) {
            const int q = guess < n - 1 ? guess : n - 2;
            i0 = q > 0 ? q - 1 : 0; i1 = q; i2 = q + 1; i3 = q + 2 < n ? q + 2 : n - 1;
            w0 = xld(col + i0); w1 = xld(col + i1); w2 = xld(col + i2); w3 = xld(col + i3);
        }
    }
    __device__ __forceinline__ YFront front(double x, int guess) const {
        YFront f;
        f.bad = a > 0 ? !(sa > sam1) : !(sa == sa);
        const bool below = x < s0, above = !below & (x > sN);
        const int p = i1;
        const bool c0 = (w1 <= x) & (x < w2);
        const bool cp = !c0 & (p + 2 < n) & (w2 <= x) & (x < w3);
        const bool cm = !c0 & !cp & (p > 0) & (w0 <= x) & (x < w1);
        f.slow = !below & !above & ((guess < 0) | !(c0 | cp | cm));
        f.where = below ? Y_BELOW : (above ? Y_ABOVE : Y_INSIDE);
        f.i = c0 ? p : (cp ? p + 1 : p - 1);
        f.si = c0 ? w1 : (cp ? w2 : w0);
        f.sj = c0 ? w2 : (cp ? w3 : w1);
        return f;
    }
    __device__ __forceinline__ double column_z() const { return ze; }
    __device__ __forceinline__ double operator[](int i) const {
        if (i == a) return sa;
        if (i == a - 1) return sam1;
        if (i == i1) return w1;
        if (i == i2) return w2;
        if (i == i0) return w0;
        if (i == i3) return w3;
        if (i == 0) return s0;
        if (i == n - 1) return sN;
        return xld(p + i);
    }
};

template <> struct YFrontOf<XKnots> { static constexpr bool value = HANK_XBACK_FRONT != 0; };
template <> struct YColumnZOf<XKnots> { static constexpr bool value = HANK_XBACK_ZREG != 0; };

__device__ __forceinline__ double xwave_sum(double v) {
#pragma unroll
    for (int off = 32; off > 0; off >>= 1) v += __shfl_xor(v, off, 64);
    return v;
}

template <int CTRL, int RM, int BM>
__device__ __forceinline__ double xdpp(double v) {
    const int lo = __builtin_amdgcn_update_dpp(0, __double2loint(v), CTRL, RM, BM, false);
    const int hi = __builtin_amdgcn_update_dpp(0, __double2hiint(v), CTRL, RM, BM, false);
    return __hiloint2double(hi, lo);
}
__device__ __forceinline__ double xwave_reduce63(double v) {
    double s = v + xdpp<0x111, 0xf, 0xf>(v);
    s = s + xdpp<0x112, 0xf, 0xf>(v);
    s = s + xdpp<0x113, 0xf, 0xf>(v);
    s = s + xdpp<0x114, 0xf, 0xe>(s);
    s = s + xdpp<0x118, 0xf, 0xc>(s);
    s = s + xdpp<0x142, 0xa, 0xf>(s);
    s = s + xdpp<0x143, 0xc, 0xf>(s);
    return s;
}

template <int SL>
__device__ __forceinline__ void xtile_store(double *t, const double *v) {
    if (SL == 1) { t[0] = v[0]; return; }
#pragma unroll
    for (int q = 0; q < SL / 2; q++) reinterpret_cast<double2 *>(t)[q] = make_double2(v[2 * q], v[2 * q + 1]);
}
template <int SL, int NS>
__device__ __forceinline__ void xtile_store_n(double *t, const double *v) {
    if (SL == 1) { t[0] = v[0]; return; }
#pragma unroll
    for (int q = 0; q < NS / 2; q++) reinterpret_cast<double2 *>(t)[q] = make_double2(v[2 * q], v[2 * q + 1]);
    if (NS & 1) t[NS - 1] = v[NS - 1];
}
template <int SL, int NS, bool FMA = false>
__device__ __forceinline__ void xtile_mix(const double *tl, const double *P, int ps, int ne, double *out) {
    const int ks = 64 * SL;
#pragma unroll 4
    for (int k = 0; k < ne; k++) {
        double v[SL];
        if (SL == 1) v[0] = tl[(size_t)k * ks];
        else {
#pragma unroll
            for (int q = 0; q < (NS + 1) / 2; q++) { const double2 d = reinterpret_cast<const double2 *>(tl + (size_t)k * ks)[q]; v[2 * q] = d.x; v[2 * q + 1] = d.y; }
        }
        const double p = P[k * ps];
#pragma unroll
        for (int q = 0; q < NS; q++) out[q] = k == 0 ? p * v[q] : (FMA ? __builtin_fma(p, v[q], out[q]) : out[q] + p * v[q]);
    }
}

template <int SL, int NS, bool FMA = false>
__device__ __forceinline__ void xtile_mix_reg(const double *tl, const double (&pr)[16], int ne, double *out) {
    const int ks = 64 * SL;
#pragma unroll
    for (int k = 0; k < 16; k++) {
        if (k < ne) {
            double v[SL];
            if (SL == 1) v[0] = tl[(size_t)k * ks];
            else {
#pragma unroll
                for (int q = 0; q < (NS + 1) / 2; q++) { const double2 d = reinterpret_cast<const double2 *>(tl + (size_t)k * ks)[q]; v[2 * q] = d.x; v[2 * q + 1] = d.y; }
            }
#pragma unroll
            for (int q = 0; q < NS; q++) out[q] = k == 0 ? pr[k] * v[q] : (FMA ? __builtin_fma(pr[k], v[q], out[q]) : out[q] + pr[k] * v[q]);
        }
    }
}

struct XBackArgs {
    Consts c;
    const double *ss_value;
    const double *xhh;
    const double *rho;
    XSync *sy;
    double *st_s;
    int *err;
    Record R;
};

template <int MAXT>
__global__ void __launch_bounds__(MAXT) k_xprimal_back(XBackArgs A) {
    extern __shared__ __attribute__((aligned(16))) double xl[];
    const Consts &c = A.c;
    const int ne = c.n_e, na = c.n_a, P = c.P, G = c.G;
    double *Vsh = xl;
    double *Pish = Vsh + (size_t)ne * 64;
    double *ash = Pish + ne * ne;
    double *xsh = ash + na;
    int *ctl = reinterpret_cast<int *>(xsh + 4 * (size_t)P);
    const XGroup g = xgroup_join(A.sy, ctl);
    if (!g.ok) return;
    const int x = g.x, cW = g.c;
    if (x != 0) return;
    const int Sact = (na + XRW - 1) / XRW;
    if (g.S < Sact) { if (threadIdx.x == 0) xfail(A.sy, XERR_PLACEMENT, x); return; }
    if (cW >= Sact) return;
    const int lane = threadIdx.x & 63, wv = __builtin_amdgcn_readfirstlane((int)(threadIdx.x >> 6));
    const bool syncw = wv >= ne;
    const bool sync_duty = blockDim.x > 64 * ne ? syncw : wv == 0;
    const int e = syncw ? 0 : wv;
    const int a = cW * XRW + lane;
    const bool own = !syncw && lane < XRW && a < na;
    const size_t pt = (size_t)e * na + (own ? a : 0);
    for (int k = threadIdx.x; k < ne * ne; k += blockDim.x) Pish[k] = c.Pi[k];
    for (int k = threadIdx.x; k < na; k += blockDim.x) ash[k] = c.a[k];
    for (int k = threadIdx.x; k < P; k += blockDim.x) {
        xsh[4 * k] = A.xhh[c.n_hh * k]; xsh[4 * k + 1] = A.xhh[c.n_hh * k + 1]; xsh[4 * k + 2] = hh_tr(c, A.xhh, k); xsh[4 * k + 3] = A.rho[k];
    }
    Consts cl = c;
    cl.a = ash;
    const double ze = c.z[e], xa = c.a[own ? a : 0];
    const size_t hs = (size_t)XG * G;
    double *const sS = A.st_s;
    if (!syncw) Vsh[e * 64 + lane] = own ? A.ss_value[pt] : 0.0;
    __syncthreads();
    int guess = -1;
    unsigned episode = 0;
    for (int i = 0; i <= P; i++) {
        if (i > 0) {
            const int t = P - i, cur = (i - 1) & 1;
            double V = 0.0;
            if (own) {
                XKnots kn;
                kn.preload(sS + (size_t)cur * hs + (size_t)e * na, a, na, guess, ze);
                const YOut o = egm_Y(cl, kn, a, e, xsh[4 * t], xsh[4 * t + 1], xsh[4 * t + 2], A.err, t, guess);
                guess = o.ib;
                V = o.V;
                const size_t ro = (size_t)t * G + pt;
                A.R.pol[ro] = o.g; A.R.ib[ro] = o.ib; A.R.A[ro] = o.A; A.R.B[ro] = o.B; A.R.u[ro] = o.u; A.R.v[ro] = o.v;
            }
            if (!syncw) Vsh[e * 64 + lane] = V;
            xlds_barrier();
        }
        if (i < P) {
            const int tx = P - 1 - i;
            if (own) {
                double E;
                xtile_mix<1, 1>(Vsh + lane, Pish + e, ne, ne, &E);
                const double bE = E * c.beta;
                const double ex = -1.0 / c.gamma;
                if (pow_domain_error(bE, ex)) set_err(A.err, ERR_DOMAIN, tx, e, a);
                const double cm = pow_crra(bE, ex);
                const double rho = xsh[4 * tx + 3];
                const double s1 = rho * ((cm - (xsh[4 * tx + 1] * ze + xsh[4 * tx + 2])) + xa);
                const double kc = c.diet ? diet_kc(c, s1, rho, 1.0 + xsh[4 * tx], xsh[4 * tx + 1] * ze + xsh[4 * tx + 2], xa) : rho * (c.beta * ex * (cm / bE));
                sS[(size_t)(i & 1) * hs + pt] = s1;
                A.R.s[(size_t)tx * G + pt] = s1; A.R.kc[(size_t)tx * G + pt] = kc;
            }
            episode++;
            xbar_arrive(!syncw);
            xbar_wait(A.sy, x, cW, Sact, episode, sync_duty);
        }
    }
}
static inline size_t x_lds_primal_back(const Consts &c) { return sizeof(double) * ((size_t)c.n_e * 64 + (size_t)c.n_e * c.n_e + c.n_a + 4 * (size_t)c.P) + XCTL_BYTES; }

struct XVfiArgs {
    Consts c;
    const double *V0;
    double r, w, tr;
    double tol;
    int max_iter;
    XSync *sy;
    double *st_s;
    int *err;
    double *Vout, *pol;
    int *iters;
    double *supnorm;
};

template <int MAXT>
__global__ void __launch_bounds__(MAXT) k_xvfi(XVfiArgs A) {
    extern __shared__ __attribute__((aligned(16))) double xl[];
    const Consts &c = A.c;
    const int ne = c.n_e, na = c.n_a, G = c.G;
    double *Vsh = xl;
    double *Pish = Vsh + (size_t)ne * 64;
    double *ash = Pish + ne * ne;
    double *redsh = ash + na;
    int *ctl = reinterpret_cast<int *>(redsh + 16);
    const XGroup g = xgroup_join(A.sy, ctl);
    if (!g.ok) return;
    const int x = g.x, cW = g.c;
    if (x != 0) return;
    const int Sact = (na + XRW - 1) / XRW;
    if (g.S < Sact) { if (threadIdx.x == 0) xfail(A.sy, XERR_PLACEMENT, x); return; }
    if (cW >= Sact) return;
    const int lane = threadIdx.x & 63, wv = __builtin_amdgcn_readfirstlane((int)(threadIdx.x >> 6));
    const bool syncw = wv >= ne;
    const bool sync_duty = blockDim.x > 64 * ne ? syncw : wv == 0;
    const int e = syncw ? 0 : wv;
    const int a = cW * XRW + lane;
    const bool own = !syncw && lane < XRW && a < na;
    const size_t pt = (size_t)e * na + (own ? a : 0);
    for (int k = threadIdx.x; k < ne * ne; k += blockDim.x) Pish[k] = c.Pi[k];
    for (int k = threadIdx.x; k < na; k += blockDim.x) ash[k] = c.a[k];
    Consts cl = c;
    cl.a = ash;
    const double ze = c.z[e], xa = c.a[own ? a : 0];
    const double rho = 1.0 / (1.0 + A.r);
    const size_t hs = (size_t)XG * G;
    double *const sS = A.st_s;
    double Vprev = own ? A.V0[pt] : 0.0, V = Vprev, pol = 0.0;
    if (!syncw) Vsh[e * 64 + lane] = Vprev;
    __syncthreads();
    int guess = -1, steps = 0, conv = 0;
    double gmax = 0.0;
    const __amdgpu_buffer_rsrc_t frs = __builtin_amdgcn_make_buffer_rsrc(&A.sy->flag[x][0][0], 0, 64 * 32 * 4, 0x00020000);
    unsigned episode = 0;
    for (int i = 0; i <= A.max_iter; i++) {
        double dmax = 0.0;
        if (i > 0) {
            const int cur = (i - 1) & 1;
            if (own) {
                XKnots kn;
                kn.preload(sS + (size_t)cur * hs + (size_t)e * na, a, na, guess, ze);
                const YOut o = egm_Y(cl, kn, a, e, A.r, A.w, A.tr, A.err, 0, guess);
                guess = o.ib;
                V = o.V; pol = o.g;
                dmax = fabs(V - Vprev);
// ... 237 lines not shown
__global__ void __launch_bounds__(MAXT) k_xtan_back(XTanBackArgs A) {
    constexpr int SL = XTileT<D>::SL;
    extern __shared__ __attribute__((aligned(16))) double xl[];
    const Consts &c = A.c;
    const Record &R = A.R;
    const int ne = c.n_e, na = c.n_a, P = c.P, G = c.G;
    double *tile = xl;
    double *rhosh = tile + (size_t)SL * ne * 64;
    double *pxsh = rhosh + ((P + 1) & ~1);
    double *dxsh = pxsh + 3 * (size_t)P + (P & 1);
    int *srcsh = reinterpret_cast<int *>(dxsh + (size_t)P * 3 * D);
    int *ctl = srcsh + P;
    const XGroup g = xgroup_join(A.sy, ctl);
    if (!g.ok) return;
    const int x = g.x, cW = g.c;
    if (x >= A.groups) return;
    const int Sact = (na + XRW - 1) / XRW;
    if (g.S < Sact) { if (threadIdx.x == 0) xfail(A.sy, XERR_PLACEMENT, x); return; }
    if (cW >= Sact) return;
    for (int k = threadIdx.x; k < P; k += blockDim.x) rhosh[k] = A.rho[k];
    for (int k = threadIdx.x; k < P; k += blockDim.x) { pxsh[3 * k] = 1.0 + A.xhh[c.n_hh * k]; pxsh[3 * k + 1] = A.xhh[c.n_hh * k + 1]; pxsh[3 * k + 2] = hh_tr(c, A.xhh, k); }
    for (int k = threadIdx.x; k < P; k += blockDim.x) srcsh[k] = A.src ? A.src[(size_t)k * Sact + cW] : ((Sact - 1) << 8);
    for (int k = threadIdx.x; k < P * D; k += blockDim.x) {
        const int t_ = k / D, d_ = k - t_ * D;
        const bool on = x * D + d_ < A.N;
        const size_t ix = (size_t)t_ * A.Ntot + A.n0 + x * D + d_;
        dxsh[(t_ * 3 + 0) * D + d_] = on ? A.dxr[ix] : 0.0;
        dxsh[(t_ * 3 + 1) * D + d_] = on ? A.dxw[ix] : 0.0;
        dxsh[(t_ * 3 + 2) * D + d_] = (on && c.n_hh > 2) ? A.dxt[ix] : 0.0;
    }
    const int lane = threadIdx.x & 63, wv = __builtin_amdgcn_readfirstlane((int)(threadIdx.x >> 6));
    const bool syncw = wv >= ne;
    const bool sync_duty = blockDim.x > 64 * ne ? syncw : wv == 0;
    const int e = syncw ? 0 : wv;
    const int r0 = cW * XRW, a = r0 + lane;
    const bool own = !syncw && lane < XRW && a < na;
    const size_t pt = (size_t)e * na + (own ? a : 0);
    const double ze = c.z[e], xa = c.a[own ? a : 0];
    const size_t hs = (size_t)XG * G;
    XRows<D> rows;
    rows.init(A.st_ds, 2 * hs);
    const size_t gx = (size_t)x * G;
    double *const myt = tile + ((size_t)e * 64 + lane) * SL;
    {
        double z[D];
#pragma unroll
        for (int k = 0; k < D; k++) z[k] = 0.0;
        if (!syncw) xtile_store_n<SL, D>(myt, z);
    }
    __syncthreads();
    double pr[16];
#pragma unroll
    for (int k = 0; k < 16; k++) pr[k] = k < ne ? c.Pi[e + ne * k] : 0.0;
    int ibY = 0;
    double cA = 0.0, cB = 0.0, cu = 0.0, cv = 0.0, ck = 0.0, cs = 0.0;
    if (own) { cs = R.s[(size_t)(P - 1) * G + pt]; if (!c.diet) ck = R.kc[(size_t)(P - 1) * G + pt]; }
    int n_ib = 0;
    double n_A = 0.0, n_B = 0.0, n_u = 0.0, n_v = 0.0, n_k = 0.0, n_s = 0.0;
    auto load_next = [&](int ty) {
        if (own && ty >= 0) {
            const size_t ro = (size_t)ty * G + pt;
            n_ib = R.ib[ro]; n_A = R.A[ro]; n_B = R.B[ro]; n_u = R.u[ro];
            if (!c.diet) n_v = R.v[ro];
            if (ty > 0) { n_s = R.s[ro - G]; if (!c.diet) n_k = R.kc[ro - G]; }
        }
    };
    constexpr bool DEEP = D <= 2;
    if constexpr (DEEP) load_next(P - 1);
    const int son = (x == 0 && cW < 32) ? cW : -1;
    (void)son;
    for (int i = 0; i <= P; i++) {
        XSTAMP(0, son, i, 0);
        if (i > 0) {
            const int t = P - i, cur = (i - 1) & 1;
            if (sync_duty) xpoll(A.sy, x, srcsh[t] & 255, srcsh[t] >> 8, (unsigned)i);
            xlds_barrier();
            XSTAMP(0, son, i, 1);
            double dV[D];
#pragma unroll
            for (int k = 0; k < D; k++) dV[k] = 0.0;
            if (own) {
                double d0[D], d1[D], dg[D];
#pragma unroll
                for (int k = 0; k < D; k++) d0[k] = d1[k] = 0.0;
                if (cA != 0.0 || cB != 0.0) {
                    const size_t rb = (size_t)cur * hs + gx + (size_t)e * na;
                    rows.load(rb + ibY, d0);
                    rows.load(rb + ibY + 1, d1);
                }
                const double cvt = c.diet ? diet_v(c, cu, pxsh[3 * t]) : cv;
#pragma unroll
                for (int k = 0; k < D; k++) {
                    const double dr = dxsh[(t * 3 + 0) * D + k], dw = dxsh[(t * 3 + 1) * D + k], dtr = dxsh[(t * 3 + 2) * D + k];
                    dg[k] = cA * d0[k] + cB * d1[k];
                    dV[k] = cu * dr + cvt * ((xa * dr + (ze * dw + dtr)) - dg[k]);
                }
                xstore_row<D>(A.dpol + (((size_t)t * A.groups + x) * G + pt) * D, dg);
            }
            if (!syncw) xtile_store_n<SL, D>(myt, dV);
            XSTAMP(0, son, i, 2);
            XSTAMPV(0, son, i);
            if (sync_duty) xpoll(A.sy, x, 0, Sact - 1, (unsigned)i);
            xlds_barrier();
            XSTAMP(0, son, i, 3);
        }
        if (i < P) {
            const int tx = P - 1 - i;
            if (own) {
                const double rho = rhosh[tx];
                const double ckt = c.diet ? diet_kc(c, cs, rho, pxsh[3 * tx], pxsh[3 * tx + 1] * ze + pxsh[3 * tx + 2], xa) : ck;
                double mx[D], ds[D];
                xtile_mix_reg<SL, D>(tile + (size_t)lane * SL, pr, ne, mx);
#pragma unroll
                for (int k = 0; k < D; k++) {
                    const double dr1 = dxsh[(tx * 3 + 0) * D + k], dw1 = dxsh[(tx * 3 + 1) * D + k], dt1 = dxsh[(tx * 3 + 2) * D + k];
                    ds[k] = ckt * mx[k] - rho * ((ze * dw1 + dt1) + cs * dr1);
                }
                rows.store((size_t)(i & 1) * hs + gx + pt, ds);
            }
            XSTAMP(0, son, i, 4);
            xbar_arrive(!syncw);
            XSTAMP(0, son, i, 5);
            if (sync_duty && !(A.stall && x == 0 && cW == 0 && i > 2)) xpublish(A.sy, x, cW, (unsigned)(i + 1));
            if constexpr (DEEP) {
                ibY = n_ib; cA = n_A; cB = n_B; cu = n_u; cv = n_v;
                if (tx > 0) { cs = n_s; ck = n_k; }
                load_next(tx - 1);
            } else if (own) {
                const size_t ro = (size_t)tx * G + pt;
                ibY = R.ib[ro]; cA = R.A[ro]; cB = R.B[ro]; cu = R.u[ro];
                if (!c.diet) cv = R.v[ro];
                if (tx > 0) { cs = R.s[ro - G]; if (!c.diet) ck = R.kc[ro - G]; }
            }
        }
    }
}
static inline size_t x_lds_tan_back(const Consts &c, int D) { return sizeof(double) * ((size_t)xtile_sl(D) * c.n_e * 64 + c.P + 1 + 3 * (size_t)c.P + 1 + 3 * (size_t)c.P * D) + sizeof(int) * (size_t)c.P + XCTL_BYTES; }

template <int NSL> struct XSlots {
    static constexpr int SP = NSL == 1 ? 1 : ((NSL + 1) / 2) * 2;
    static constexpr int SL = NSL <= 2 ? NSL : (NSL <= 6 ? 6 : 10);
};
struct XSlotsRt { int SP, SL; };
template <int NSL> constexpr XSlotsRt xslots_of() { return {XSlots<NSL>::SP, XSlots<NSL>::SL}; }
static inline XSlotsRt xslots(int NSL) { return NSL == 1 ? xslots_of<1>() : NSL == 2 ? xslots_of<2>() : NSL == 3 ? xslots_of<3>() : NSL == 4 ? xslots_of<4>() : xslots_of<5>(); }

struct XDualBackArgs {
    XBackArgs p;
    const double *dxr, *dxw, *dxt;
    int Ntot, n0, N;
    double *st_ds;
    double *dpol;
    int groups;
};

template <int D, int MAXT>
__global__ void __launch_bounds__(MAXT) k_xdual_back(XDualBackArgs B) {
    constexpr int NSL = D + 1, SL = XSlots<NSL>::SL, IV = D;
    extern __shared__ __attribute__((aligned(16))) double xl[];
    const XBackArgs &A = B.p;
    const Consts &c = A.c;
    const int ne = c.n_e, na = c.n_a, P = c.P, G = c.G;
    double *tile = xl;
    double *ash = tile + (size_t)SL * ne * 64;
    double *xsh = ash + ((na + 1) & ~1);
    double *dxsh = xsh + 4 * (size_t)P;
    int *ctl = reinterpret_cast<int *>(dxsh + (size_t)P * 3 * D);
#ifdef HANK_XSTAMP
    const unsigned long long t_entry = __builtin_amdgcn_s_memrealtime();
#endif
    const XGroup g = xgroup_join(A.sy, ctl);
    if (!g.ok) return;
    const int x = g.x, cW = g.c;
    if (x >= B.groups) return;
    const int Sact = (na + XRW - 1) / XRW;
    if (g.S < Sact) { if (threadIdx.x == 0) xfail(A.sy, XERR_PLACEMENT, x); return; }
    if (cW >= Sact) return;
    const int son = (x == 0 && cW < 32) ? cW : -1;
    (void)son;
#ifdef HANK_XSTAMP
    if (son >= 0 && threadIdx.x == 0) g_xstamps[0][son][0][8] = t_entry;
#endif
    XSTAMP1(0, son, 9);
    const int lane = threadIdx.x & 63, wv = __builtin_amdgcn_readfirstlane((int)(threadIdx.x >> 6));
    const bool syncw = wv >= ne;
    const bool sync_duty = blockDim.x > 64 * ne ? syncw : wv == 0;
    const int e = syncw ? 0 : wv;
    const int a = cW * XRW + lane;
    const bool own = !syncw && lane < XRW && a < na;
    const int ng = B.groups;
    const bool rc0 = 0 % ng == x, rc1 = 1 % ng == x, rc2 = 2 % ng == x, rc3 = 3 % ng == x, rc4 = 4 % ng == x, rc5 = 5 % ng == x, rc6 = 6 % ng == x, rc7 = 7 % ng == x;
    const size_t pt = (size_t)e * na + (own ? a : 0);
    for (int k = threadIdx.x; k < na; k += blockDim.x) ash[k] = c.a[k];
    for (int k = threadIdx.x; k < P; k += blockDim.x) {
        xsh[4 * k] = A.xhh[c.n_hh * k]; xsh[4 * k + 1] = A.xhh[c.n_hh * k + 1]; xsh[4 * k + 2] = hh_tr(c, A.xhh, k); xsh[4 * k + 3] = A.rho[k];
    }
    for (int k = threadIdx.x; k < P * D; k += blockDim.x) {
        const int t_ = k / D, d_ = k - t_ * D;
        const bool on = x * D + d_ < B.N;
        const size_t ix = (size_t)t_ * B.Ntot + B.n0 + x * D + d_;
        dxsh[(t_ * 3 + 0) * D + d_] = on ? B.dxr[ix] : 0.0;
        dxsh[(t_ * 3 + 1) * D + d_] = on ? B.dxw[ix] : 0.0;
        dxsh[(t_ * 3 + 2) * D + d_] = (on && c.n_hh > 2) ? B.dxt[ix] : 0.0;
    }
    Consts cl = c;
    cl.a = ash;
    const double ze = c.z[e], xa = c.a[own ? a : 0];
    const size_t hs = (size_t)XG * G, gx = (size_t)x * G;
    double *const sS = A.st_s;
    XRows<D> rows;
    rows.init(B.st_ds, 2 * hs);
    double *const myt = tile + ((size_t)e * 64 + lane) * SL;
    if (!syncw) {
        double z[NSL];
#pragma unroll
        for (int k = 0; k < D; k++) z[k] = 0.0;
        z[IV] = own ? A.ss_value[pt] : 0.0;
        xtile_store_n<SL, NSL>(myt, z);
    }
    __syncthreads();
    double pr[16];
#pragma unroll
    for (int k = 0; k < 16; k++) pr[k] = k < ne ? c.Pi[e + ne * k] : 0.0;
    int guess = -1;
    unsigned episode = 0;
    XSTAMP1(0, son, 10);
    for (int i = 0; i <= P; i++) {
        XSTAMP(0, son, i, 0);
        if (i > 0) {
            const int t = P - i, cur = (i - 1) & 1;
            double tv[NSL];
#pragma unroll
            for (int k = 0; k < NSL; k++) tv[k] = 0.0;
            if (own) {
                XKnots kn;
                kn.preload(sS + (size_t)cur * hs + gx + (size_t)e * na, a, na, guess, ze);
                const size_t rb = (size_t)cur * hs + gx + (size_t)e * na;
                const int q = guess < 0 ? 0 : (guess < na - 1 ? guess : na - 2);
                double w0[D], w1[D];
                rows.load(rb + q, w0);
                rows.load(rb + q + 1, w1);
                const YOut o = egm_Y(cl, kn, a, e, xsh[4 * t], xsh[4 * t + 1], xsh[4 * t + 2], A.err, t, guess);
                guess = o.ib;
                tv[IV] = o.V;
                XSTAMP(0, son, i, 1);
                double d0[D], d1[D], dg[D];
#pragma unroll
                for (int k = 0; k < D; k++) d0[k] = d1[k] = 0.0;
                if (o.A != 0.0 || o.B != 0.0) {
                    if (o.ib == q) {
#pragma unroll
                        for (int k = 0; k < D; k++) { d0[k] = w0[k]; d1[k] = w1[k]; }
                    } else if (o.ib == q + 1) {
#pragma unroll
                        for (int k = 0; k < D; k++) d0[k] = w1[k];
                        rows.load(rb + o.ib + 1, d1);
                    } else if (o.ib == q - 1) {
#pragma unroll
                        for (int k = 0; k < D; k++) d1[k] = w0[k];
                        rows.load(rb + o.ib, d0);
                    } else {
                        rows.load(rb + o.ib, d0);
                        rows.load(rb + o.ib + 1, d1);
                    }
                }
#pragma unroll
                for (int k = 0; k < D; k++) {
                    const double dr = dxsh[(t * 3 + 0) * D + k], dw = dxsh[(t * 3 + 1) * D + k], dtr = dxsh[(t * 3 + 2) * D + k];
                    dg[k] = o.A * d0[k] + o.B * d1[k];
                    tv[k] = o.u * dr + o.v * ((xa * dr + (ze * dw + dtr)) - dg[k]);
                }
                xstore_row<D>(B.dpol + (((size_t)t * B.groups + x) * G + pt) * D, dg);
                const size_t ro = (size_t)t * G + pt;
                if (rc0) A.R.pol[ro] = o.g;
                if (rc1) A.R.ib[ro] = o.ib;
                if (rc2) A.R.A[ro] = o.A;
                if (rc3) A.R.B[ro] = o.B;
                if (rc4) A.R.u[ro] = o.u;
                if (rc5) A.R.v[ro] = o.v;
            }
            if (!syncw) xtile_store_n<SL, NSL>(myt, tv);
            XSTAMP(0, son, i, 2);
            XSTAMPV(0, son, i);
            xlds_barrier();
            XSTAMP(0, son, i, 3);
        }
        if (i < P) {
            const int tx = P - 1 - i;
            if (own) {
                double mx[NSL];
                xtile_mix_reg<SL, NSL>(tile + (size_t)lane * SL, pr, ne, mx);
                const double bE = mx[IV] * c.beta;
                const double ex = -1.0 / c.gamma;
                if (pow_domain_error(bE, ex)) set_err(A.err, ERR_DOMAIN, tx, e, a);
                const double cm = pow_crra(bE, ex);
                const double rho = xsh[4 * tx + 3];
                const double s1 = rho * ((cm - (xsh[4 * tx + 1] * ze + xsh[4 * tx + 2])) + xa);
                const double kc = c.diet ? diet_kc(c, s1, rho, 1.0 + xsh[4 * tx], xsh[4 * tx + 1] * ze + xsh[4 * tx + 2], xa) : rho * (c.beta * ex * (cm / bE));
                double ds[D];
#pragma unroll
                for (int k = 0; k < D; k++) {
                    const double dr1 = dxsh[(tx * 3 + 0) * D + k], dw1 = dxsh[(tx * 3 + 1) * D + k], dt1 = dxsh[(tx * 3 + 2) * D + k];
                    ds[k] = kc * mx[k] - rho * ((ze * dw1 + dt1) + s1 * dr1);
                }
                sS[(size_t)(i & 1) * hs + gx + pt] = s1;
                rows.store((size_t)(i & 1) * hs + gx + pt, ds);
                if (rc6) A.R.s[(size_t)tx * G + pt] = s1;
                if (rc7) A.R.kc[(size_t)tx * G + pt] = kc;
            }
            episode++;
            XSTAMP(0, son, i, 4);
            xbar_arrive(!syncw);
            XSTAMP(0, son, i, 5);
            xbar_wait(A.sy, x, cW, Sact, episode, sync_duty);
        }
    }
    XSTAMP1(0, son, 11);
}
static inline size_t x_lds_dual_back(const Consts &c, int D) { return sizeof(double) * ((size_t)xslots(D + 1).SL * c.n_e * 64 + c.n_a + 1 + 4 * (size_t)c.P + 3 * (size_t)c.P * D) + XCTL_BYTES; }

#ifndef HANK_XPRIMAL_LWG_IN_SWEEP
#define HANK_XPRIMAL_LWG_IN_SWEEP 1
#endif
constexpr int XUCAP = 64;
struct XSweepFwdArgs {
    Consts c;
    Record R;
    XSync *sy;
    double *st;
    const double *D0;
    const double *dpol;
    int groups;
    double *Dvirt;
    double *aggpart;
    double *daggpart;
    const int *src;
    const int *overflow;
    const int2 *units;
    int all_members;
};

template <int D, bool VAL, int MAXT>
__global__ void __launch_bounds__(MAXT) k_xfwd(XSweepFwdArgs A) {
#pragma clang fp contract(fast)
    constexpr int NSL = D + (VAL ? 1 : 0);
    constexpr int SP = XSlots<NSL>::SP, SL = XSlots<NSL>::SL;
    constexpr int IV = D;
    constexpr int DD = D > 0 ? D : 1;
    constexpr bool PIREG = NSL < 4;
    extern __shared__ __attribute__((aligned(16))) double xl[];
    const Consts &c = A.c;
    const Record &R = A.R;
    const int ne = c.n_e, na = c.n_a, P = c.P, G = c.G;
    double *tile = xl;
    double *Pish = tile + (size_t)SL * ne * 64;
    constexpr int NAP = 2 * NSL;
    double *aggsh = Pish + ((ne * ne + 1) & ~1);
    int *closh = reinterpret_cast<int *>(aggsh + (size_t)ne * 64 * NAP);
    int *srcsh = closh + (size_t)P * ne;
    int *ctl = srcsh + P;
    if (*A.overflow) return;
    const XGroup g = xgroup_join(A.sy, ctl);
    if (!g.ok) return;
    const int x = g.x, cW = g.c;
    if (x >= A.groups) return;
    const int Sact = (na + XRW - 1) / XRW;
    if (g.S < Sact) { if (threadIdx.x == 0) xfail(A.sy, XERR_PLACEMENT, x); return; }
    if (cW >= Sact) return;
    constexpr bool RECL = VAL && D == 0 && HANK_XPRIMAL_LWG_IN_SWEEP;
    const bool recD = VAL && x == 0, recL = RECL && x == 1 % A.groups;
    for (int k = threadIdx.x; k < ne * ne; k += blockDim.x) Pish[k] = c.Pi[k];
    for (int k = threadIdx.x; k < P * ne; k += blockDim.x) closh[k] = R.clo[k];
    for (int k = threadIdx.x; k < P; k += blockDim.x) {
        int w = A.src[(size_t)k * Sact + cW];
        if (A.all_members || (recL && ((w >> 17) & 1))) w = (w & ~0xffff) | ((Sact - 1) << 8);
        srcsh[k] = w;
    }
    const int lane = threadIdx.x & 63, wv = __builtin_amdgcn_readfirstlane((int)(threadIdx.x >> 6));
    const bool syncw = wv >= ne;
    const bool sync_duty = blockDim.x > 64 * ne ? syncw : wv == 0;
    const int e = syncw ? 0 : wv;
    const int r0 = cW * XRW, r = r0 + lane;
    const bool own = !syncw && lane < XRW && r < na;
    const bool virt = !syncw && lane == 63;
    const bool live = own || virt;
    const size_t pt = (size_t)e * na + (own ? r : 0);
    const double xar = c.a[own ? r : 0];
    const size_t GM = (size_t)ne * Sact * 64;
    const size_t gx = (size_t)x * GM;
    const size_t slot = gx + ((size_t)e * Sact + cW) * 64 + lane;
    const size_t hs = (size_t)XG * GM;
    double pr[16];
#pragma unroll
    for (int k = 0; k < 16; k++) pr[k] = (PIREG && k < ne) ? c.Pi[ne * e + k] : 0.0;
    XRows<SP> rows;
    rows.init(A.st, 2 * hs);
    double *const myt = tile + ((size_t)e * 64 + lane) * SL;
    double mxp[NSL];
#pragma unroll
    for (int k = 0; k < NSL; k++) mxp[k] = 0.0;
    if constexpr (VAL) { if (own) mxp[IV] = A.D0[pt]; }
    {
        double sv[SP];
#pragma unroll
        for (int k = 0; k < SP; k++) sv[k] = k < NSL ? mxp[k] : 0.0;
        if (live) rows.store(slot, sv);
    }
    double polr = 0.0, Dr = 0.0, lwr = 0.0, igr = 0.0, dpr[DD];
#pragma unroll
    for (int k = 0; k < DD; k++) dpr[k] = 0.0;
#ifdef HANK_X_TIMING_L2
#define XTPER(bit, t) ((((HANK_X_TIMING_L2) >> (bit)) & 1) ? ((t) & 1) : (t))
#else
#define XTPER(bit, t) (t)
#endif
    auto prefetch = [&](int t_) {
        const int t = XTPER(2, t_);
        const size_t ro = (size_t)t * G + (size_t)e * na + (own ? r : 0);
        polr = R.pol[ro];
        if constexpr (D > 0) xload_row_plain<DD>(A.dpol + ((size_t)t * A.groups + x) * (size_t)G * D + ((size_t)e * na + (own ? r : 0)) * D, dpr);
        if constexpr (RECL) { lwr = R.lw[ro]; igr = R.ig[ro]; }
        else if constexpr (!VAL && D > 0) Dr = R.Dseq[ro + G];
    };
    int2 ud[2];
    int qlo[2];
    double qw[2], qg[2], qdn[2], qdp[2][DD], dd[2][SP];
    bool qon[2], qvl[2];
    const int2 *const ubase = A.units + (size_t)cW * XUCAP;
    auto unit_desc = [&](int t, int u) -> int2 {
        const int2 q = ubase[(size_t)XTPER(3, t) * Sact * XUCAP + u];
        return make_int2(__builtin_amdgcn_readfirstlane(q.x), __builtin_amdgcn_readfirstlane(q.y));
    };
    auto load_rec = [&](auto U, int t_, int2 d, int i0) {
        constexpr int u = decltype(U)::value;
        const int t = XTPER(0, t_), tp = XTPER(1, t_);
        (void)tp;
        const int ue = d.x & 15, ja = (d.x >> 4) & 0xfff, cnt = (d.x >> 16) & 0xfff, nv = (d.y >> 16) & 0xff;
        const int i = i0 + lane;
        const bool real = i < cnt;
        qvl[u] = !real && i < cnt + nv;
        qon[u] = real || qvl[u];
        const size_t cb = (size_t)t * G + (size_t)ue * na;
        const int j = real ? ja + i : (qvl[u] ? 0 : min(ja + max(cnt - 1, 0), na - 1));
        qlo[u] = R.lo[cb + j];
        if constexpr (VAL) { qw[u] = R.lw[cb + j]; if constexpr (D > 0) qg[u] = R.ig[cb + j]; }
        else { const double2 wg = R.lwg[cb + j]; qw[u] = wg.x; qg[u] = wg.y; if constexpr (D > 0) qdn[u] = R.Dseq[cb + G + j]; }
        if constexpr (D > 0) xload_row_plain<DD>(A.dpol + (((size_t)tp * A.groups + x) * G + (size_t)ue * na + j) * D, qdp[u]);
    };
    auto load_state = [&](auto U, size_t hb, int2 d, int i0) {
        constexpr int u = decltype(U)::value;
        const int ue = d.x & 15, ja = (d.x >> 4) & 0xfff, cnt = (d.x >> 16) & 0xfff;
#pragma unroll
        for (int k = 0; k < SP; k++) dd[u][k] = 0.0;
        const int i = i0 + lane, j = ja + i;
        const size_t row = qvl[u] ? ((size_t)ue * Sact + (i - cnt)) * 64 + 63 : ((size_t)ue * Sact + j / XRW) * 64 + j % XRW;
        if (qon[u]) rows.load(hb + gx + row, dd[u]);
    };
    const std::integral_constant<int, 0> I0;
    const std::integral_constant<int, 1> I1;
    int2 udn[2];
    bool udv[2] = {false, false};
    udn[0] = udn[1] = make_int2(0, 0);
    auto request_units = [&](int t) {
        const int tc = min(t, P - 1), tu = XTPER(3, tc);
        int nu = (srcsh[tu] >> 18) & 0xff;
        nu = t < P ? nu : 0;
        udv[0] = wv < nu; udv[1] = wv + ne < nu;
        udn[0] = ubase[(size_t)tu * Sact * XUCAP + (udv[0] ? wv : 0)];
        udn[1] = ubase[(size_t)tu * Sact * XUCAP + (udv[1] ? wv + ne : 0)];
    };
    auto take_units = [&]() {
        ud[0] = udv[0] ? make_int2(__builtin_amdgcn_readfirstlane(udn[0].x), __builtin_amdgcn_readfirstlane(udn[0].y)) : make_int2(0, 0);
        ud[1] = udv[1] ? make_int2(__builtin_amdgcn_readfirstlane(udn[1].x), __builtin_amdgcn_readfirstlane(udn[1].y)) : make_int2(0, 0);
    };
    constexpr int DPI = D == 0 ? 0 : (D <= 2 ? 1 : D / 2);
    constexpr int XFWD_NLD = 1 + DPI + (RECL ? 2 : ((!VAL && D > 0) ? 1 : 0));
    auto next_units_loads = [&](int t) {
        const int t1 = min(t + 1, P - 1);
        load_rec(I0, t1, ud[0], 0);
        load_rec(I1, t1, ud[1], 0);
        request_units(t + 2);
    };
    auto next_period_loads = [&](int t) {
        prefetch(min(t + 1, P - 1));
    };
    xbar_arrive(!syncw);
    if (sync_duty) xpublish(A.sy, x, cW, 1u);
    ud[0] = ud[1] = make_int2(0, 0);
    if (!syncw) { request_units(0); take_units(); load_rec(I0, 0, ud[0], 0); load_rec(I1, 0, ud[1], 0); prefetch(0); request_units(1); }
    int cur = 0;
    bool vnz = false;
    const int son = (x == 0 && cW < 32) ? cW : -1;
    (void)son;
    auto reduce_agg = [&](int tp) {
        const double *ap = aggsh + (size_t)lane * NAP;
        double sk[NAP];
#pragma unroll
        for (int k = 0; k < NAP; k++) sk[k] = 0.0;
        for (int k2 = 0; k2 < ne; k2++) {
            double v[NAP];
            if (NAP == 1) v[0] = ap[(size_t)k2 * 64 * NAP];
            else {
#pragma unroll
                for (int q = 0; q < NAP / 2; q++) { const double2 d = reinterpret_cast<const double2 *>(ap + (size_t)k2 * 64 * NAP)[q]; v[2 * q] = d.x; v[2 * q + 1] = d.y; }
            }
#pragma unroll
            for (int k = 0; k < NAP; k++) sk[k] += v[k];
        }
        const size_t pb = (size_t)tp * Sact + cW;
#pragma unroll
        for (int k = 0; k < D; k++) {
            const double pd = xwave_reduce63(sk[k]), pd2 = xwave_reduce63(sk[NSL + k]);
            if (lane == 63) { A.daggpart[pb * (size_t)(2 * XG * D) + x * D + k] = pd; A.daggpart[pb * (size_t)(2 * XG * D) + XG * D + x * D + k] = pd2; }
        }
        if constexpr (VAL) {
            if (recD) {
                const double pD = xwave_reduce63(sk[IV]), pD2 = xwave_reduce63(sk[NSL + IV]);
                if (lane == 63) { A.aggpart[2 * pb] = pD; A.aggpart[2 * pb + 1] = pD2; }
            }
        }
    };
    for (int t = 0; t < P; t++) {
        XSTAMP(1, son, t, 0);
        const size_t base = (size_t)t * G + (size_t)e * na;
        const size_t hb = (size_t)cur * hs;
        const int sw = srcsh[t];
        int clo = 0;
        if (!syncw) {
            clo = min(max(closh[t * ne + e], 0), na);
            double z[SL];
#pragma unroll
            for (int k = 0; k < SL; k++) z[k] = 0.0;
            xtile_store<SL>(myt, z);
        }
        if (sync_duty) xpoll(A.sy, x, sw & 255, (sw >> 8) & 255, (unsigned)(t + 1));
        xlds_barrier();
        XSTAMP(1, son, t, 1);
        if (sync_duty && t > 0) reduce_agg(t - 1);
        double pagg[DD];
#pragma unroll
        for (int k = 0; k < DD; k++) pagg[k] = 0.0;
        double v0 = 0.0;
        if (!syncw) {
            const bool need0 = recL && r0 == 0 && vnz && clo == 0;
            if constexpr (RECL) {
                if (need0 && lane < Sact) v0 = rows.load_one(hb + gx + ((size_t)e * Sact + lane) * 64 + 63, IV);
            }
            load_state(I0, hb, ud[0], 0);
            load_state(I1, hb, ud[1], 0);
#ifdef HANK_DEV_NOATOMIC
#define lds_add(p, v) (*(p) = (v))
#endif
            auto process_pc = [&](auto U, int2 d) {
                constexpr int u = decltype(U)::value;
                const int ta = d.y & 0xff, tb = (d.y >> 8) & 0xff;
                double *const colt = tile + (size_t)(d.x & 15) * 64 * SL;
                const double w = qw[u], w1 = 1.0 - w;
                double gD = qg[u], Dv = 0.0;
                if constexpr (VAL) { Dv = dd[u][IV]; gD = qg[u] * Dv; }
                else { if (qvl[u]) gD = 0.0; }
                const int tl = qlo[u] - r0, th = tl + 1;
                const bool doL = qon[u] && tl >= ta && tl < tb, doH = qon[u] && th >= ta && th < tb;
                const int thp = __builtin_amdgcn_update_dpp(-2, doH ? th : -2, 0x138, 0xf, 0xf, false);
                const bool take = doL && thp == tl;
                const bool given = __builtin_amdgcn_update_dpp(0, take ? 1 : 0, 0x130, 0xf, 0xf, false) != 0;
                double *const tpl = colt + (size_t)(doL ? tl : 0) * SL, *const tph = colt + (size_t)(doH ? th : 0) * SL;
#pragma unroll
                for (int k = 0; k < D; k++) {
                    const double hk = w * dd[u][k] + gD * qdp[u][k];
                    const double hp = xdpp<0x138, 0xf, 0xf>(hk);
                    const double lk = w1 * dd[u][k] - gD * qdp[u][k];
                    if (doL) lds_add(tpl + k, take ? lk + hp : lk);
                    if (doH && !given) lds_add(tph + k, hk);
                }
                if constexpr (VAL) {
                    if (doL) lds_add(tpl + IV, w1 * Dv);
                    if (doH) lds_add(tph + IV, w * Dv);
                }
                if constexpr (!VAL) {
                    if (doL && !qvl[u]) {
#pragma unroll
                        for (int k = 0; k < D; k++) pagg[k] += qdp[u][k] * qdn[u];
                    }
                }
            };
            auto process_1 = [&](auto U, int2 d) {
                constexpr int u = decltype(U)::value;
                if (!qon[u]) return;
                const int ta = d.y & 0xff, tb = (d.y >> 8) & 0xff;
                double *const colt = tile + (size_t)(d.x & 15) * 64 * SL;
                const double w = qw[u], w1 = 1.0 - w;
                double gD = qg[u], Dv = 0.0;
                if constexpr (VAL) { Dv = dd[u][IV]; gD = qg[u] * Dv; }
                else { if (qvl[u]) gD = 0.0; }
                const int tl = qlo[u] - r0, th = tl + 1;
                if (tl >= ta && tl < tb) {
                    double *tp = colt + (size_t)tl * SL;
#pragma unroll
                    for (int k = 0; k < D; k++) lds_add(tp + k, w1 * dd[u][k] - gD * qdp[u][k]);
                    if constexpr (VAL) lds_add(tp + IV, w1 * Dv);
                    if constexpr (!VAL) {
                        if (!qvl[u]) {
#pragma unroll
                            for (int k = 0; k < D; k++) pagg[k] += qdp[u][k] * qdn[u];
                        }
                    }
                }
                if (th >= ta && th < tb) {
                    double *tp = colt + (size_t)th * SL;
#pragma unroll
                    for (int k = 0; k < D; k++) lds_add(tp + k, w * dd[u][k] + gD * qdp[u][k]);
                    if constexpr (VAL) lds_add(tp + IV, w * Dv);
                }
            };
            constexpr bool PRECOMB = HANK_XFWD_PRECOMBINE && (D + (VAL ? 1 : 0)) >= 3;
            auto process = [&](auto U, int2 d) { if constexpr (PRECOMB) process_pc(U, d); else process_1(U, d); };
            process(I0, ud[0]);
            process(I1, ud[1]);
#ifdef HANK_DEV_NOATOMIC
#undef lds_add
#endif
#ifdef HANK_X_TIMING_L2
            const int nu = (srcsh[XTPER(3, t)] >> 18) & 0xff;
#else
            const int nu = (sw >> 18) & 0xff;
#endif
            for (int u2 = wv; u2 < nu; u2 += ne) {
                const int2 d = u2 < 2 * ne ? ud[u2 >= ne ? 1 : 0] : unit_desc(t, u2);
                const int tot = ((d.x >> 16) & 0xfff) + ((d.y >> 16) & 0xff);
                for (int i0 = u2 < 2 * ne ? 64 : 0; i0 < tot; i0 += 64) {
                    load_rec(I0, t, d, i0);
                    load_state(I0, hb, d, i0);
                    process(I0, d);
                }
            }
            if constexpr (RECL) { if (need0) v0 = xwave_sum(v0); }
            take_units();
            XSTAMP(1, son, t, 2);
            double cT[NSL];
#pragma unroll
            for (int k = 0; k < NSL; k++) cT[k] = ((own && r < clo) || (virt && clo > 0 && vnz)) ? mxp[k] : 0.0;
            if (clo > r0) {
#pragma unroll
                for (int k = 0; k < NSL; k++) cT[k] = xwave_reduce63(cT[k]);
            }
            if (virt) xtile_store_n<SL, NSL>(myt, cT);
        }
        XSTAMP(1, son, t, 3);
        XSTAMPV(1, son, t);
        if (sync_duty) xpoll(A.sy, x, 0, Sact - 1, (unsigned)(t + 1));
        xlds_barrier();
        XSTAMP(1, son, t, 4);
        vnz = ((sw >> 16) & 1) != 0;
        const int nxt = cur ^ 1;
        if (!syncw) {
            next_units_loads(t);
            double mx[NSL];
            if (PIREG) xtile_mix_reg<SL, NSL, true>(tile + (size_t)lane * SL, pr, ne, mx);
            else xtile_mix<SL, NSL, true>(tile + (size_t)lane * SL, Pish + ne * e, 1, ne, mx);
            if (live) {
                double sv[SP];
#pragma unroll
                for (int k = 0; k < SP; k++) sv[k] = k < NSL ? mx[k] : 0.0;
                rows.store((size_t)nxt * hs + slot, sv);
            }
            double at[NAP];
#pragma unroll
            for (int k = 0; k < NAP; k++) at[k] = 0.0;
            if constexpr (RECL) {
                if (recL && own) {
                    double Dfull = mxp[IV];
                    if (r == 0 && clo == 0) Dfull += v0;
                    R.lwg[base + r] = make_double2(lwr, igr * Dfull);
                }
            }
            if constexpr (VAL) {
                if (recD) {
                    if (own) R.Dseq[(size_t)(t + 1) * G + pt] = mx[IV];
                    else if (virt) A.Dvirt[((size_t)t * ne + e) * 64 + cW] = mx[IV];
                    at[IV] = live ? polr * mx[IV] : 0.0;
                    at[NSL + IV] = live ? xar * mx[IV] : 0.0;
                }
            }
#pragma unroll
            for (int k = 0; k < D; k++) {
                double term = live ? polr * mx[k] : 0.0;
                if constexpr (VAL) term = live ? (polr * mx[k] + dpr[k] * mx[IV]) : 0.0;
                else term = (term + pagg[k]) + ((own && r < clo) ? dpr[k] * Dr : 0.0);
                at[k] = term;
                at[NSL + k] = live ? xar * mx[k] : 0.0;
            }
            xtile_store<NAP>(aggsh + ((size_t)e * 64 + lane) * NAP, at);
#pragma unroll
            for (int k = 0; k < NSL; k++) mxp[k] = mx[k];
        }
        cur = nxt;
        XSTAMP(1, son, t, 5);
        if (!syncw) {
            asm volatile("; XFWD_BATCH_BEGIN" ::: "memory");
            next_period_loads(t);
            XSTAMP(1, son, t, 7);
            asm volatile("; XFWD_BATCH_END\n\ts_waitcnt vmcnt(%0)" ::"n"(XFWD_NLD) : "memory");
            XSTAMP(1, son, t, 8);
        }
        xlds_barrier();
        if (sync_duty) xpublish(A.sy, x, cW, (unsigned)(t + 2));
        XSTAMP(1, son, t, 6);
    }
    if (sync_duty) reduce_agg(P - 1);
}
static inline size_t x_lds_fwd(const Consts &c, int D, bool val) {
    const int NSL = D + (val ? 1 : 0), NAP = 2 * NSL;
    return sizeof(double) * ((size_t)xslots(NSL).SL * c.n_e * 64 + (size_t)c.n_e * c.n_e + 1 + (size_t)c.n_e * 64 * NAP) + sizeof(int) * ((size_t)c.P * c.n_e + c.P) + XCTL_BYTES;
}

__global__ void k_xunits_fwd(Consts c, Record R, int Sact, int *src, int2 *units, int *overflow, int ucap) {
    __shared__ int2 su[16][XUCAP];
    __shared__ int scnt[16], slo, shi, sany0;
    __shared__ int sst[16][XRW + 3];
    const int t = blockIdx.x, m = blockIdx.y, ne = c.n_e, na = c.n_a;
    const int r0 = m * XRW, nrows = min(XRW, na - r0);
    __shared__ int sclo[16], sclop[16], soff[17];
    if (threadIdx.x == 0) { slo = m; shi = m; sany0 = 0; }
    if ((int)threadIdx.x < ne) {
        sclo[threadIdx.x] = R.clo[(size_t)t * ne + threadIdx.x];
        sclop[threadIdx.x] = t > 0 ? R.clo[(size_t)(t - 1) * ne + threadIdx.x] : 0;
    }
    for (int k = threadIdx.x; k < ne * (XRW + 3); k += blockDim.x) {
        const int e = k / (XRW + 3), q = k - e * (XRW + 3);
        sst[e][q] = min(max(R.start[((size_t)t * ne + e) * (na + 1) + min(max(r0 - 1 + q, 0), na)], 0), na);
    }
    __syncthreads();
    bool vnz = false;
    for (int e = 0; e < ne; e++) vnz = vnz || sclop[e] > 0;
    const int lane = threadIdx.x & 63, wave = threadIdx.x >> 6, nwaves = blockDim.x >> 6;
    for (int e = wave; e < ne; e += nwaves) {
        const int clo = sclo[e];
        auto S = [&](int rr) { return sst[e][min(max(rr - (r0 - 1), 0), XRW + 2)]; };
        auto lanes_of = [&](int a, int b, int *ja_out, bool *has0_out) {
            const int ja = S(r0 + a - 1 < 0 ? 0 : r0 + a - 1);
            const bool has0 = ja == 0 && clo <= 0 && vnz;
            const int cnt = max(S(r0 + b) - ja, 0);
            *ja_out = ja; *has0_out = has0;
            return cnt;
        };
        int nxt = nrows;
        if (lane < nrows) {
            int ja; bool has0;
            (void)lanes_of(lane, lane + 1, &ja, &has0);
            auto fits = [&](int b) { const int c2 = max(S(r0 + b) - ja, 0); return c2 + ((has0 && c2 > 0) ? Sact : 0) <= 64; };
            int lo = lane + 1, hi = nrows;
            if (lo < hi && fits(lo + 1)) {
                if (fits(hi)) lo = hi;
                else {
                    lo = lo + 1;
                    while (hi - lo > 1) { const int mid = (lo + hi) >> 1; if (fits(mid)) lo = mid; else hi = mid; }
                }
            }
            nxt = lo;
        }
        int n = 0, ta = 0;
        while (ta < nrows && n < XUCAP) {
            const int tb = __shfl(nxt, ta, 64);
            int ja; bool has0;
            const int cnt = lanes_of(ta, tb, &ja, &has0);
            const int nv = (has0 && cnt > 0) ? Sact : 0;
            if (cnt > 0) {
                if (lane == 0) {
                    su[e][n] = make_int2(e | (ja << 4) | (cnt << 16), ta | (tb << 8) | (nv << 16));
                    atomicMin(&slo, ja / XRW); atomicMax(&shi, (ja + cnt - 1) / XRW);
                    if (nv) sany0 = 1;
                }
                n++;
            }
            ta = tb;
        }
        if (lane == 0) {
            if (ta < nrows) atomicExch(overflow, 1);
            scnt[e] = n;
        }
    }
    __syncthreads();
    if (threadIdx.x == 0) {
        int off = 0;
        for (int e = 0; e < ne; e++) { soff[e] = off; off += scnt[e]; }
        soff[ne] = off;
    }
    __syncthreads();
    for (int k = threadIdx.x; k < min(soff[ne], XUCAP); k += blockDim.x) {
        int e = 0;
        while (e + 1 < ne && soff[e + 1] <= k) e++;
        units[((size_t)t * Sact + m) * XUCAP + k] = su[e][k - soff[e]];
    }
    if (threadIdx.x == 0) {
        int tot = soff[ne], anyclo = 0, anyopen = 0;
        for (int e = 0; e < ne; e++) {
            if (sclo[e] > 0) anyclo = 1; else anyopen = 1;
        }
        if (tot > ucap) { atomicExch(overflow, 1); tot = min(tot, XUCAP); }
        int ml = min(slo, m), mh = max(shi, m);
        if (sany0) { ml = 0; mh = Sact - 1; }
        const int allv = (m == 0 && vnz && anyopen) ? 1 : 0;
        src[(size_t)t * Sact + m] = ml | (mh << 8) | (anyclo << 16) | (allv << 17) | (tot << 18);
    }
}

__global__ void k_xsrc_back(Consts c, Record R, int Sact, int *src) {
    __shared__ int smin[256], smax[256];
    const int t = blockIdx.x, m = blockIdx.y;
    const int r0 = m * XRW, rows = min(XRW, c.n_a - r0);
    int lo = 1 << 30, hi = -1;
    for (int k = threadIdx.x; k < rows * c.n_e; k += blockDim.x) {
        const int e = k / rows, a = r0 + (k - e * rows);
        const size_t ro = (size_t)t * c.G + (size_t)e * c.n_a + a;
        if (R.A[ro] != 0.0 || R.B[ro] != 0.0) { const int ib = R.ib[ro]; lo = min(lo, ib); hi = max(hi, ib + 1); }
    }
    smin[threadIdx.x] = lo; smax[threadIdx.x] = hi;
    __syncthreads();
    if (threadIdx.x == 0) {
        for (int k = 1; k < (int)blockDim.x; k++) { lo = min(lo, smin[k]); hi = max(hi, smax[k]); }
        int ml = m, mh = m;
        if (hi >= 0) { ml = min(m, max(lo, 0) / XRW); mh = max(m, min(hi, c.n_a - 1) / XRW); }
        src[(size_t)t * Sact + m] = ml | (mh << 8);
    }
}
__global__ void k_xrho(const double *xhh, int n_hh, int P, double *rho) {
    const int t = blockIdx.x * blockDim.x + threadIdx.x;
    if (t < P) rho[t] = 1.0 / (1.0 + xhh[n_hh * t]);
}

__global__ void k_xfix_D(Consts c, double *Dseq, const double *Dvirt, int Sact, double *D0own) {
    const int idx = blockIdx.x * blockDim.x + threadIdx.x;
// ... 115 lines not shown
```

Baseline: 8083 JVPs/s.

## Use AMD buffer resource loads/stores with 32-bit offsets in dual sweep kernels

Replaces 64-bit pointer arithmetic in the dual backward and value forward sweep kernels with raw buffer load/store intrinsics. Each kernel builds buffer resource descriptors for the record slab, dpol and the state arrays, and addresses them with 32-bit vector/scalar offsets so the compiler can keep base addresses in scalar registers and use fewer VGPRs for addressing. A host check that all offsets fit in 32 bits falls back to the unfused path when they do not. The change adds complexity, and buffer bounds checking could silently mask errors if the descriptor sizes are wrong.

```diff
diff --git a/julia-newtonraphsonhank_amd/csrc/hank_hip.hip b/julia-newtonraphsonhank_amd/csrc/hank_hip.hip
--- a/julia-newtonraphsonhank_amd/csrc/hank_hip.hip
+++ b/julia-newtonraphsonhank_amd/csrc/hank_hip.hip
@@ -878,6 +878,21 @@
     }
     return HANK_OK;
 }
+static XRecOff x_rec_off(const hank_ctx *ctx) {
+    const Record &R = ctx->R;
+    const char *b = ctx->rec_slab;
+    auto off = [&](const void *p) { return (unsigned)((const char *)p - b); };
+    XRecOff o{};
+    o.rec = b; o.bytes = (unsigned)ctx->rec_bytes;
+    o.pol = off(R.pol); o.ib = off(R.ib); o.A = off(R.A); o.B = off(R.B); o.u = off(R.u); o.v = off(R.v); o.s = off(R.s); o.kc = off(R.kc);
+    o.lo = off(R.lo); o.lw = off(R.lw); o.ig = off(R.ig); o.Dseq = off(R.Dseq);
+    return o;
+}
+static bool x_dual_addr_fits(const hank_ctx *ctx) {
+    if (!HANK_XADDR_BUF) return true;
+    const Consts &c = ctx->c;
+    return x_addr_fits(ctx->rec_bytes, (unsigned long long)c.P, XG, (unsigned long long)c.G, XD_MAX, (unsigned long long)((c.n_a + XRW - 1) / XRW), XUCAP);
+}
 static int x_back(XSection &sec, XTan *dual = nullptr) {
     hank_ctx *ctx = sec.ctx; XWork &X = ctx->xw;
     const Consts &c = ctx->c;
@@ -890,6 +905,7 @@
         XDualBackArgs db{};
         db.p = ab; db.dxr = dual->dxr; db.dxw = dual->dxw; db.dxt = dual->dxt; db.Ntot = dual->N; db.n0 = ps.n0; db.N = ps.N;
         db.st_ds = X.st_ds; db.dpol = dual->dpol + ps.dpol_off; db.groups = ps.groups;
+        db.ro = x_rec_off(ctx); db.dpol_bytes = (unsigned)((size_t)c.P * ps.groups * c.G * ps.D * sizeof(double));
         x_launch_dual_back(sec, X, c, ps.D, db);
     } else x_launch_primal_back(sec, X, c, ab);
     HIPC(ctx, ctx->spans.end(PRIMAL_BACK, sec.stream(), 1));
@@ -948,6 +964,7 @@
     if (!val) { const int rc = ensure_lwg(ctx); if (rc) return rc; }
     XSweepFwdArgs fa = x_fwd_args(ctx, val);
     fa.sy = X.sync + 2 + 2 * p + 1; fa.st = X.st_dD; fa.daggpart = w->daggpart; fa.groups = ps.groups; fa.dpol = w->dpol + ps.dpol_off;
+    fa.ro = x_rec_off(ctx); fa.dpol_bytes = (unsigned)((size_t)ctx->c.P * ps.groups * ctx->c.G * ps.D * sizeof(double));
     x_launch_fwd(sec, X, ctx->c, ps.D, val, fa);
     return HANK_OK;
 }
@@ -1512,7 +1529,7 @@
     return ctx->xdual_back && x_has_dual_back(X) && 64 * (ctx->c.n_e + 1) <= X.maxt && x_lds_dual_back(ctx->c, D) <= (size_t)X.lds_max;
 }
 static bool use_x_fused(const hank_ctx *ctx, int N) {
-    if (ctx->schedule < 1 || !x_tan_fits(ctx, N)) return false;
+    if (ctx->schedule < 1 || !x_tan_fits(ctx, N) || !x_dual_addr_fits(ctx)) return false;
     if (ctx->schedule == 1) return true;
     return N <= XG * ctx->xw.dmax && x_dual_back_fits(ctx, ctx->xw.dmax);
 }
diff --git a/julia-newtonraphsonhank_amd/csrc/hank_kernels.h b/julia-newtonraphsonhank_amd/csrc/hank_kernels.h
--- a/julia-newtonraphsonhank_amd/csrc/hank_kernels.h
+++ b/julia-newtonraphsonhank_amd/csrc/hank_kernels.h
@@ -122,6 +122,59 @@
     else if (MODE == 2) __builtin_nontemporal_store(x, p);
     else *p = x;
 }
+
+typedef unsigned int wv2u __attribute__((ext_vector_type(2)));
+typedef unsigned int wv4u __attribute__((ext_vector_type(4)));
+__device__ __forceinline__ __amdgpu_buffer_rsrc_t wide_rsrc(const void *p) {
+    return __builtin_amdgcn_make_buffer_rsrc(const_cast<void *>(p), 0, 0x7fffffff, 0x00020000);
+}
+__device__ __forceinline__ double wide_ld64(__amdgpu_buffer_rsrc_t rs, int vo, int so) {
+    const wv2u q = __builtin_amdgcn_raw_buffer_load_b64(rs, vo, so, 0);
+    return __hiloint2double((int)q.y, (int)q.x);
+}
+__device__ __forceinline__ wv2u wide_ld2i(__amdgpu_buffer_rsrc_t rs, int vo, int so) { return __builtin_amdgcn_raw_buffer_load_b64(rs, vo, so, 0); }
+template <int AUX>
+__device__ __forceinline__ void wide_ld2d(__amdgpu_buffer_rsrc_t rs, int vo, int so, double &a, double &b) {
+    const wv4u q = __builtin_amdgcn_raw_buffer_load_b128(rs, vo, so, AUX);
+    a = __hiloint2double((int)q.y, (int)q.x); b = __hiloint2double((int)q.w, (int)q.z);
+}
+__device__ __forceinline__ wv4u wide_ld128(__amdgpu_buffer_rsrc_t rs, int vo, int so) { return __builtin_amdgcn_raw_buffer_load_b128(rs, vo, so, 0); }
+__device__ __forceinline__ void wide_st2d_nt(double a, double b, __amdgpu_buffer_rsrc_t rs, int vo, int so) {
+    wv4u q;
+    q.x = (unsigned)__double2loint(a); q.y = (unsigned)__double2hiint(a); q.z = (unsigned)__double2loint(b); q.w = (unsigned)__double2hiint(b);
+    __builtin_amdgcn_raw_buffer_store_b128(q, rs, vo, so, 2);
+}
+__device__ __forceinline__ void wide_st64_nt(double v, __amdgpu_buffer_rsrc_t rs, int vo, int so) {
+    wv2u q;
+    q.x = (unsigned)__double2loint(v); q.y = (unsigned)__double2hiint(v);
+    __builtin_amdgcn_raw_buffer_store_b64(q, rs, vo, so, 2);
+}
+
+__device__ __forceinline__ __amdgpu_buffer_rsrc_t buf_rsrc(const void *p, unsigned bytes) {
+    return __builtin_amdgcn_make_buffer_rsrc(const_cast<void *>(p), 0, (int)bytes, 0x00020000);
+}
+template <int AUX>
+__device__ __forceinline__ double buf_ld64(__amdgpu_buffer_rsrc_t rs, int vo, int so) {
+    const wv2u q = __builtin_amdgcn_raw_buffer_load_b64(rs, vo, so, AUX);
+    return __hiloint2double((int)q.y, (int)q.x);
+}
+template <int AUX>
+__device__ __forceinline__ int buf_ld32(__amdgpu_buffer_rsrc_t rs, int vo, int so) { return (int)__builtin_amdgcn_raw_buffer_load_b32(rs, vo, so, AUX); }
+template <int AUX>
+__device__ __forceinline__ void buf_st64(double v, __amdgpu_buffer_rsrc_t rs, int vo, int so) {
+    wv2u q;
+    q.x = (unsigned)__double2loint(v); q.y = (unsigned)__double2hiint(v);
+    __builtin_amdgcn_raw_buffer_store_b64(q, rs, vo, so, AUX);
+}
+template <int AUX>
+__device__ __forceinline__ void buf_st32(int v, __amdgpu_buffer_rsrc_t rs, int vo, int so) { __builtin_amdgcn_raw_buffer_store_b32((unsigned)v, rs, vo, so, AUX); }
+template <int AUX>
+__device__ __forceinline__ void buf_st2d(double a, double b, __amdgpu_buffer_rsrc_t rs, int vo, int so) {
+    wv4u q;
+    q.x = (unsigned)__double2loint(a); q.y = (unsigned)__double2hiint(a); q.z = (unsigned)__double2loint(b); q.w = (unsigned)__double2hiint(b);
+    __builtin_amdgcn_raw_buffer_store_b128(q, rs, vo, so, AUX);
+}
+constexpr int BUF_AUX_REC = HANK_ST_REC == 1 ? 16 : (HANK_ST_REC == 2 ? 2 : 0);
 
 __device__ __forceinline__ double mix_mul(double p, double v) { return p * v; }
 __device__ __forceinline__ double2 mix_mul(double p, double2 v) { return make_double2(p * v.x, p * v.y); }
diff --git a/julia-newtonraphsonhank_amd/csrc/hank_wide.h b/julia-newtonraphsonhank_amd/csrc/hank_wide.h
--- a/julia-newtonraphsonhank_amd/csrc/hank_wide.h
+++ b/julia-newtonraphsonhank_amd/csrc/hank_wide.h
@@ -55,32 +55,6 @@
     __builtin_amdgcn_sched_barrier(0);
 }
 
-typedef unsigned int wv2u __attribute__((ext_vector_type(2)));
-typedef unsigned int wv4u __attribute__((ext_vector_type(4)));
-__device__ __forceinline__ __amdgpu_buffer_rsrc_t wide_rsrc(const void *p) {
-    return __builtin_amdgcn_make_buffer_rsrc(const_cast<void *>(p), 0, 0x7fffffff, 0x00020000);
-}
-__device__ __forceinline__ double wide_ld64(__amdgpu_buffer_rsrc_t rs, int vo, int so) {
-    const wv2u q = __builtin_amdgcn_raw_buffer_load_b64(rs, vo, so, 0);
-    return __hiloint2double((int)q.y, (int)q.x);
-}
-__device__ __forceinline__ wv2u wide_ld2i(__amdgpu_buffer_rsrc_t rs, int vo, int so) { return __builtin_amdgcn_raw_buffer_load_b64(rs, vo, so, 0); }
-template <int AUX>
-__device__ __forceinline__ void wide_ld2d(__amdgpu_buffer_rsrc_t rs, int vo, int so, double &a, double &b) {
-    const wv4u q = __builtin_amdgcn_raw_buffer_load_b128(rs, vo, so, AUX);
-    a = __hiloint2double((int)q.y, (int)q.x); b = __hiloint2double((int)q.w, (int)q.z);
-}
-__device__ __forceinline__ wv4u wide_ld128(__amdgpu_buffer_rsrc_t rs, int vo, int so) { return __builtin_amdgcn_raw_buffer_load_b128(rs, vo, so, 0); }
-__device__ __forceinline__ void wide_st2d_nt(double a, double b, __amdgpu_buffer_rsrc_t rs, int vo, int so) {
-    wv4u q;
-    q.x = (unsigned)__double2loint(a); q.y = (unsigned)__double2hiint(a); q.z = (unsigned)__double2loint(b); q.w = (unsigned)__double2hiint(b);
-    __builtin_amdgcn_raw_buffer_store_b128(q, rs, vo, so, 2);
-}
-__device__ __forceinline__ void wide_st64_nt(double v, __amdgpu_buffer_rsrc_t rs, int vo, int so) {
-    wv2u q;
-    q.x = (unsigned)__double2loint(v); q.y = (unsigned)__double2hiint(v);
-    __builtin_amdgcn_raw_buffer_store_b64(q, rs, vo, so, 2);
-}
 
 #ifdef HANK_WIDE_TIMING_L2
 #define WIDE_TPER(t) ((t) & 1)
diff --git a/julia-newtonraphsonhank_amd/csrc/hank_xaddr.h b/julia-newtonraphsonhank_amd/csrc/hank_xaddr.h
--- /dev/null
+++ b/julia-newtonraphsonhank_amd/csrc/hank_xaddr.h
@@ -0,0 +1,12 @@
+#pragma once
+
+namespace hank {
+
+constexpr unsigned long long XADDR_MARGIN = 1ull << 24;
+static inline bool x_addr_fits(unsigned long long rec_bytes, unsigned long long P, unsigned long long groups, unsigned long long G, unsigned long long D,
+                               unsigned long long members, unsigned long long ucap) {
+    const unsigned long long lim = (1ull << 32) - XADDR_MARGIN;
+    return rec_bytes <= lim && P * groups * G * D * 8ull <= lim && P * members * ucap * 8ull <= lim && G * D * 8ull <= XADDR_MARGIN;
+}
+
+}
diff --git a/julia-newtonraphsonhank_amd/csrc/hank_xsweep.h b/julia-newtonraphsonhank_amd/csrc/hank_xsweep.h
--- a/julia-newtonraphsonhank_amd/csrc/hank_xsweep.h
+++ b/julia-newtonraphsonhank_amd/csrc/hank_xsweep.h
@@ -8,7 +8,11 @@
 #ifndef HANK_XBACK_ZREG
 #define HANK_XBACK_ZREG 1
 #endif
+#ifndef HANK_XADDR_BUF
+#define HANK_XADDR_BUF 1
+#endif
 #include "hank_kernels.h"
+#include "hank_xaddr.h"
 #include <type_traits>
 
 namespace hank {
@@ -64,6 +68,31 @@
     __device__ __forceinline__ double load_one(size_t row, int k) const {
         return D == 1 ? xld(base + row) : xld(base + ((size_t)(k / 2) * plane + row) * 2 + (k & 1));
     }
+    static constexpr int RB = D == 1 ? 8 : 16;
+    __device__ __forceinline__ void init_buf(double *p, int rows_total) {
+        base = p; plane = (size_t)rows_total;
+        rs = __builtin_amdgcn_make_buffer_rsrc(p, 0, rows_total * 8 * D, 0x00020000);
+    }
+    __device__ __forceinline__ void load_vs(int rv, int rs_, double *v) const {
+        if (D == 1) {
+            v[0] = buf_ld64<16>(rs, rv * RB, rs_ * RB);
+        } else {
+#pragma unroll
+            for (int k = 0; k < D / 2; k++) {
+                const xv4u q = __builtin_amdgcn_raw_buffer_load_b128(rs, rv * RB, (k * (int)plane + rs_) * RB, 16);
+                v[2 * k] = __hiloint2double((int)q.y, (int)q.x);
+                v[2 * k + 1] = __hiloint2double((int)q.w, (int)q.z);
+            }
+        }
+    }
+    __device__ __forceinline__ void store_vs(int rv, int rs_, const double *v) const {
+        if (D == 1) {
+            buf_st64<0>(v[0], rs, rv * RB, rs_ * RB);
+        } else {
+#pragma unroll
+            for (int k = 0; k < D / 2; k++) buf_st2d<0>(v[2 * k], v[2 * k + 1], rs, rv * RB, (k * (int)plane + rs_) * RB);
+        }
+    }
     __device__ __forceinline__ void store(size_t row, const double *v) const {
         if (D == 1) {
             base[row] = v[0];
@@ -84,6 +113,24 @@
     }
 }
 template <int D>
+__device__ __forceinline__ void xstore_row_buf(__amdgpu_buffer_rsrc_t rs, int vo, int so, const double *v) {
+    if (D == 1) {
+        buf_st64<2>(v[0], rs, vo, so);
+    } else {
+#pragma unroll
+        for (int k = 0; k < D / 2; k++) buf_st2d<2>(v[2 * k], v[2 * k + 1], rs, vo + 16 * k, so);
+    }
+}
+template <int D>
+__device__ __forceinline__ void xload_row_buf(__amdgpu_buffer_rsrc_t rs, int vo, int so, double *v) {
+    if (D == 1) {
+        v[0] = buf_ld64<0>(rs, vo, so);
+    } else {
+#pragma unroll
+        for (int k = 0; k < D / 2; k++) wide_ld2d<0>(rs, vo + 16 * k, so, v[2 * k], v[2 * k + 1]);
+    }
+}
+template <int D>
 __device__ __forceinline__ void xload_row_plain(const double *p, double *v) {
     if (D == 1) {
         v[0] = *p;
@@ -92,6 +139,8 @@
         for (int k = 0; k < D / 2; k++) { const double2 q = reinterpret_cast<const double2 *>(p)[k]; v[2 * k] = q.x; v[2 * k + 1] = q.y; }
     }
 }
+
+__device__ __forceinline__ int xopaque(int v) { asm volatile("" : "+s"(v)); return v; }
 
 struct XGroup { int x, c, S, ok; };
 
@@ -210,11 +259,18 @@
     if ((threadIdx.x & 63) == 0) *reinterpret_cast<volatile unsigned *>(&sy->flag[x][c][0]) = episode;
 }
 
-struct XKnots {
+template <bool BUF>
+struct XKnotsT {
     const double *p;
+    __amdgpu_buffer_rsrc_t rs;
+    int so;
     int a, n, i0, i1, i2, i3;
     double sa, sam1, s0, sN, w0, w1, w2, w3;
     double ze;
+    __device__ __forceinline__ double ld(int i) const {
+        if constexpr (BUF) return buf_ld64<16>(rs, i * 8, so);
+        else return xld(p + i);
+    }
     __device__ __forceinline__ void preload(const double *col, int a_, int n_, int guess, double ze_) {
         p = col; a = a_; n = n_; ze = ze_;
         sa = xld(col + a);
@@ -227,6 +283,20 @@
             const int q = guess < n - 1 ? guess : n - 2;
             i0 = q > 0 ? q - 1 : 0; i1 = q; i2 = q + 1; i3 = q + 2 < n ? q + 2 : n - 1;
             w0 = xld(col + i0); w1 = xld(col + i1); w2 = xld(col + i2); w3 = xld(col + i3);
+        }
+    }
+    __device__ __forceinline__ void preload(__amdgpu_buffer_rsrc_t rs_, int so_, int a_, int n_, int guess, double ze_) {
+        rs = rs_; so = so_; a = a_; n = n_; ze = ze_;
+        sa = ld(a);
+        sam1 = ld(a > 0 ? a - 1 : 0);
+        s0 = ld(0);
+        sN = ld(n - 1);
+        i0 = i1 = i2 = i3 = -1;
+        w0 = w1 = w2 = w3 = 0.0;
+        if (guess >= 0) {
+            const int q = guess < n - 1 ? guess : n - 2;
+            i0 = q > 0 ? q - 1 : 0; i1 = q; i2 = q + 1; i3 = q + 2 < n ? q + 2 : n - 1;
+            w0 = ld(i0); w1 = ld(i1); w2 = ld(i2); w3 = ld(i3);
         }
     }
     __device__ __forceinline__ YFront front(double x, int guess) const {
@@ -254,12 +324,13 @@
         if (i == i3) return w3;
         if (i == 0) return s0;
         if (i == n - 1) return sN;
-        return xld(p + i);
+        return ld(i);
     }
 };
-
-template <> struct YFrontOf<XKnots> { static constexpr bool value = HANK_XBACK_FRONT != 0; };
-template <> struct YColumnZOf<XKnots> { static constexpr bool value = HANK_XBACK_ZREG != 0; };
+using XKnots = XKnotsT<false>;
+
+template <bool BUF> struct YFrontOf<XKnotsT<BUF>> { static constexpr bool value = HANK_XBACK_FRONT != 0; };
+template <bool BUF> struct YColumnZOf<XKnotsT<BUF>> { static constexpr bool value = HANK_XBACK_ZREG != 0; };
 
 __device__ __forceinline__ double xwave_sum(double v) {
 #pragma unroll
@@ -314,12 +385,13 @@
     }
 }
 
-template <int SL, int NS, bool FMA = false>
+template <int SL, int NS, bool FMA = false, bool BRK = false>
 __device__ __forceinline__ void xtile_mix_reg(const double *tl, const double (&pr)[16], int ne, double *out) {
     const int ks = 64 * SL;
 #pragma unroll
     for (int k = 0; k < 16; k++) {
-        if (k < ne) {
+        if (BRK && k > 0 && k >= ne) break;
+        if (BRK || k < ne) {
             double v[SL];
             if (SL == 1) v[0] = tl[(size_t)k * ks];
             else {
@@ -331,6 +403,12 @@
         }
     }
 }
+
+struct XRecOff {
+    const char *rec;
+    unsigned bytes;
+    unsigned pol, ib, A, B, u, v, s, kc, lo, lw, ig, Dseq;
+};
 
 struct XBackArgs {
     Consts c;
@@ -874,11 +952,14 @@
     double *st_ds;
     double *dpol;
     int groups;
+    XRecOff ro;
+    unsigned dpol_bytes;
 };
 
 template <int D, int MAXT>
 __global__ void __launch_bounds__(MAXT) k_xdual_back(XDualBackArgs B) {
     constexpr int NSL = D + 1, SL = XSlots<NSL>::SL, IV = D;
+    constexpr bool XB = HANK_XADDR_BUF != 0;
     extern __shared__ __attribute__((aligned(16))) double xl[];
     const XBackArgs &A = B.p;
     const Consts &c = A.c;
@@ -931,7 +1012,11 @@
     const size_t hs = (size_t)XG * G, gx = (size_t)x * G;
     double *const sS = A.st_s;
     XRows<D> rows;
-    rows.init(B.st_ds, 2 * hs);
+    if constexpr (XB) rows.init_buf(B.st_ds, 2 * XG * G); else rows.init(B.st_ds, 2 * hs);
+    __amdgpu_buffer_rsrc_t rrec, rdp, rkn;
+    if constexpr (XB) { rrec = buf_rsrc(B.ro.rec, B.ro.bytes); rdp = buf_rsrc(B.dpol, B.dpol_bytes); rkn = buf_rsrc(sS, (unsigned)(2 * hs * 8)); }
+    const int ipt = (int)pt, igx = x * G, ihs = XG * G;
+    const int rcm0 = __builtin_amdgcn_readfirstlane((rc0 ? 1 : 0) | (rc1 ? 2 : 0) | (rc2 ? 4 : 0) | (rc3 ? 8 : 0) | (rc4 ? 16 : 0) | (rc5 ? 32 : 0) | (rc6 ? 64 : 0) | (rc7 ? 128 : 0));
     double *const myt = tile + ((size_t)e * 64 + lane) * SL;
     if (!syncw) {
         double z[NSL];
@@ -955,13 +1040,15 @@
 #pragma unroll
             for (int k = 0; k < NSL; k++) tv[k] = 0.0;
             if (own) {
-                XKnots kn;
-                kn.preload(sS + (size_t)cur * hs + gx + (size_t)e * na, a, na, guess, ze);
+                XKnotsT<XB> kn;
+                const int icb = cur * ihs + igx + e * na;
+                if constexpr (XB) kn.preload(rkn, icb * 8, a, na, guess, ze);
+                else kn.preload(sS + (size_t)cur * hs + gx + (size_t)e * na, a, na, guess, ze);
                 const size_t rb = (size_t)cur * hs + gx + (size_t)e * na;
                 const int q = guess < 0 ? 0 : (guess < na - 1 ? guess : na - 2);
                 double w0[D], w1[D];
-                rows.load(rb + q, w0);
-                rows.load(rb + q + 1, w1);
+                if constexpr (XB) { rows.load_vs(q, icb, w0); rows.load_vs(q + 1, icb, w1); }
+                else { rows.load(rb + q, w0); rows.load(rb + q + 1, w1); }
                 const YOut o = egm_Y(cl, kn, a, e, xsh[4 * t], xsh[4 * t + 1], xsh[4 * t + 2], A.err, t, guess);
                 guess = o.ib;
                 tv[IV] = o.V;
@@ -976,14 +1063,14 @@
                     } else if (o.ib == q + 1) {
 #pragma unroll
                         for (int k = 0; k < D; k++) d0[k] = w1[k];
-                        rows.load(rb + o.ib + 1, d1);
+                        if constexpr (XB) rows.load_vs(o.ib + 1, icb, d1); else rows.load(rb + o.ib + 1, d1);
                     } else if (o.ib == q - 1) {
 #pragma unroll
                         for (int k = 0; k < D; k++) d1[k] = w0[k];
-                        rows.load(rb + o.ib, d0);
+                        if constexpr (XB) rows.load_vs(o.ib, icb, d0); else rows.load(rb + o.ib, d0);
                     } else {
-                        rows.load(rb + o.ib, d0);
-                        rows.load(rb + o.ib + 1, d1);
+                        if constexpr (XB) { rows.load_vs(o.ib, icb, d0); rows.load_vs(o.ib + 1, icb, d1); }
+                        else { rows.load(rb + o.ib, d0); rows.load(rb + o.ib + 1, d1); }
                     }
                 }
 #pragma unroll
@@ -992,14 +1079,25 @@
                     dg[k] = o.A * d0[k] + o.B * d1[k];
                     tv[k] = o.u * dr + o.v * ((xa * dr + (ze * dw + dtr)) - dg[k]);
                 }
-                xstore_row<D>(B.dpol + (((size_t)t * B.groups + x) * G + pt) * D, dg);
-                const size_t ro = (size_t)t * G + pt;
-                if (rc0) A.R.pol[ro] = o.g;
-                if (rc1) A.R.ib[ro] = o.ib;
-                if (rc2) A.R.A[ro] = o.A;
-                if (rc3) A.R.B[ro] = o.B;
-                if (rc4) A.R.u[ro] = o.u;
-                if (rc5) A.R.v[ro] = o.v;
+                if constexpr (XB) {
+                    xstore_row_buf<D>(rdp, ipt * (8 * D), (int)((unsigned)((t * B.groups + x) * G) * (unsigned)(8 * D)), dg);
+                    const int tg = t * G, rcm = xopaque(rcm0);
+                    if (rcm & 1) buf_st64<BUF_AUX_REC>(o.g, rrec, ipt * 8, (int)(B.ro.pol + (unsigned)tg * 8u));
+                    if (rcm & 2) buf_st32<BUF_AUX_REC>(o.ib, rrec, ipt * 4, (int)(B.ro.ib + (unsigned)tg * 4u));
+                    if (rcm & 4) buf_st64<BUF_AUX_REC>(o.A, rrec, ipt * 8, (int)(B.ro.A + (unsigned)tg * 8u));
+                    if (rcm & 8) buf_st64<BUF_AUX_REC>(o.B, rrec, ipt * 8, (int)(B.ro.B + (unsigned)tg * 8u));
+                    if (rcm & 16) buf_st64<BUF_AUX_REC>(o.u, rrec, ipt * 8, (int)(B.ro.u + (unsigned)tg * 8u));
+                    if (rcm & 32) buf_st64<BUF_AUX_REC>(o.v, rrec, ipt * 8, (int)(B.ro.v + (unsigned)tg * 8u));
+                } else {
+                    xstore_row<D>(B.dpol + (((size_t)t * B.groups + x) * G + pt) * D, dg);
+                    const size_t ro = (size_t)t * G + pt;
+                    if (rc0) A.R.pol[ro] = o.g;
+                    if (rc1) A.R.ib[ro] = o.ib;
+                    if (rc2) A.R.A[ro] = o.A;
+                    if (rc3) A.R.B[ro] = o.B;
+                    if (rc4) A.R.u[ro] = o.u;
+                    if (rc5) A.R.v[ro] = o.v;
+                }
             }
             if (!syncw) xtile_store_n<SL, NSL>(myt, tv);
             XSTAMP(0, son, i, 2);
@@ -1011,7 +1109,7 @@
             const int tx = P - 1 - i;
             if (own) {
                 double mx[NSL];
-                xtile_mix_reg<SL, NSL>(tile + (size_t)lane * SL, pr, ne, mx);
+                xtile_mix_reg<SL, NSL, false, XB>(tile + (size_t)lane * SL, pr, XB ? xopaque(ne) : ne, mx);
                 const double bE = mx[IV] * c.beta;
                 const double ex = -1.0 / c.gamma;
                 if (pow_domain_error(bE, ex)) set_err(A.err, ERR_DOMAIN, tx, e, a);
@@ -1025,10 +1123,18 @@
                     const double dr1 = dxsh[(tx * 3 + 0) * D + k], dw1 = dxsh[(tx * 3 + 1) * D + k], dt1 = dxsh[(tx * 3 + 2) * D + k];
                     ds[k] = kc * mx[k] - rho * ((ze * dw1 + dt1) + s1 * dr1);
                 }
-                sS[(size_t)(i & 1) * hs + gx + pt] = s1;
-                rows.store((size_t)(i & 1) * hs + gx + pt, ds);
-                if (rc6) A.R.s[(size_t)tx * G + pt] = s1;
-                if (rc7) A.R.kc[(size_t)tx * G + pt] = kc;
+                if constexpr (XB) {
+                    const int ihb = (i & 1) * ihs + igx, rcm = xopaque(rcm0);
+                    buf_st64<0>(s1, rkn, ipt * 8, ihb * 8);
+                    rows.store_vs(ipt, ihb, ds);
+                    if (rcm & 64) buf_st64<BUF_AUX_REC>(s1, rrec, ipt * 8, (int)(B.ro.s + (unsigned)(tx * G) * 8u));
+                    if (rcm & 128) buf_st64<BUF_AUX_REC>(kc, rrec, ipt * 8, (int)(B.ro.kc + (unsigned)(tx * G) * 8u));
+                } else {
+                    sS[(size_t)(i & 1) * hs + gx + pt] = s1;
+                    rows.store((size_t)(i & 1) * hs + gx + pt, ds);
+                    if (rc6) A.R.s[(size_t)tx * G + pt] = s1;
+                    if (rc7) A.R.kc[(size_t)tx * G + pt] = kc;
+                }
             }
             episode++;
             XSTAMP(0, son, i, 4);
@@ -1060,6 +1166,8 @@
     const int *overflow;
     const int2 *units;
     int all_members;
+    XRecOff ro;
+    unsigned dpol_bytes;
 };
 
 template <int D, bool VAL, int MAXT>
@@ -1070,6 +1178,7 @@
     constexpr int IV = D;
     constexpr int DD = D > 0 ? D : 1;
     constexpr bool PIREG = NSL < 4;
+    constexpr bool XB = HANK_XADDR_BUF != 0 && VAL && D > 0;
     extern __shared__ __attribute__((aligned(16))) double xl[];
     const Consts &c = A.c;
     const Record &R = A.R;
@@ -1116,7 +1225,11 @@
 #pragma unroll
     for (int k = 0; k < 16; k++) pr[k] = (PIREG && k < ne) ? c.Pi[ne * e + k] : 0.0;
     XRows<SP> rows;
-    rows.init(A.st, 2 * hs);
+    const int iGM = ne * Sact * 64;
+    if constexpr (XB) rows.init_buf(A.st, 2 * XG * iGM); else rows.init(A.st, 2 * hs);
+    __amdgpu_buffer_rsrc_t rrec, rdp;
+    if constexpr (XB) { rrec = buf_rsrc(A.ro.rec, A.ro.bytes); rdp = buf_rsrc(A.dpol, A.dpol_bytes); }
+    const int ipt = e * na + (own ? r : 0), igx = x * iGM, ihs = XG * iGM, islot = (e * Sact + cW) * 64;
     double *const myt = tile + ((size_t)e * 64 + lane) * SL;
     double mxp[NSL];
 #pragma unroll
@@ -1126,7 +1239,8 @@
         double sv[SP];
 #pragma unroll
         for (int k = 0; k < SP; k++) sv[k] = k < NSL ? mxp[k] : 0.0;
-        if (live) rows.store(slot, sv);
+        if constexpr (XB) { if (live) rows.store_vs(lane, igx + islot, sv); }
+        else if (live) rows.store(slot, sv);
     }
     double polr = 0.0, Dr = 0.0, lwr = 0.0, igr = 0.0, dpr[DD];
 #pragma unroll
@@ -1138,6 +1252,11 @@
 #endif
     auto prefetch = [&](int t_) {
         const int t = XTPER(2, t_);
+        if constexpr (XB) {
+            polr = buf_ld64<0>(rrec, ipt * 8, (int)(A.ro.pol + (unsigned)(t * G) * 8u));
+            xload_row_buf<DD>(rdp, ipt * (8 * D), (int)((unsigned)((t * A.groups + x) * G) * (unsigned)(8 * D)), dpr);
+            return;
+        }
         const size_t ro = (size_t)t * G + (size_t)e * na + (own ? r : 0);
         polr = R.pol[ro];
         if constexpr (D > 0) xload_row_plain<DD>(A.dpol + ((size_t)t * A.groups + x) * (size_t)G * D + ((size_t)e * na + (own ? r : 0)) * D, dpr);
@@ -1149,8 +1268,12 @@
     double qw[2], qg[2], qdn[2], qdp[2][DD], dd[2][SP];
     bool qon[2], qvl[2];
     const int2 *const ubase = A.units + (size_t)cW * XUCAP;
+    auto unit_ld = [&](int tu, int u) -> int2 {
+        return A.units[(unsigned)((tu * Sact + cW) * XUCAP + u)];
+    };
     auto unit_desc = [&](int t, int u) -> int2 {
-        const int2 q = ubase[(size_t)XTPER(3, t) * Sact * XUCAP + u];
+        int2 q;
+        if constexpr (XB) q = unit_ld(XTPER(3, t), u); else q = ubase[(size_t)XTPER(3, t) * Sact * XUCAP + u];
         return make_int2(__builtin_amdgcn_readfirstlane(q.x), __builtin_amdgcn_readfirstlane(q.y));
     };
     auto load_rec = [&](auto U, int t_, int2 d, int i0) {
@@ -1164,17 +1287,30 @@
         qon[u] = real || qvl[u];
         const size_t cb = (size_t)t * G + (size_t)ue * na;
         const int j = real ? ja + i : (qvl[u] ? 0 : min(ja + max(cnt - 1, 0), na - 1));
+        if constexpr (XB) {
+            const int icb = t * G + ue * na;
+            qlo[u] = buf_ld32<0>(rrec, j * 4, (int)(A.ro.lo + (unsigned)icb * 4u));
+            qw[u] = buf_ld64<0>(rrec, j * 8, (int)(A.ro.lw + (unsigned)icb * 8u));
+            qg[u] = buf_ld64<0>(rrec, j * 8, (int)(A.ro.ig + (unsigned)icb * 8u));
+            xload_row_buf<DD>(rdp, j * (8 * D), (int)((unsigned)((tp * A.groups + x) * G + ue * na) * (unsigned)(8 * D)), qdp[u]);
+            return;
+        }
         qlo[u] = R.lo[cb + j];
         if constexpr (VAL) { qw[u] = R.lw[cb + j]; if constexpr (D > 0) qg[u] = R.ig[cb + j]; }
         else { const double2 wg = R.lwg[cb + j]; qw[u] = wg.x; qg[u] = wg.y; if constexpr (D > 0) qdn[u] = R.Dseq[cb + G + j]; }
         if constexpr (D > 0) xload_row_plain<DD>(A.dpol + (((size_t)tp * A.groups + x) * G + (size_t)ue * na + j) * D, qdp[u]);
     };
-    auto load_state = [&](auto U, size_t hb, int2 d, int i0) {
+    auto load_state = [&](auto U, size_t hb, int hc, int2 d, int i0) {
         constexpr int u = decltype(U)::value;
         const int ue = d.x & 15, ja = (d.x >> 4) & 0xfff, cnt = (d.x >> 16) & 0xfff;
 #pragma unroll
         for (int k = 0; k < SP; k++) dd[u][k] = 0.0;
         const int i = i0 + lane, j = ja + i;
+        if constexpr (XB) {
+            const int rowi = qvl[u] ? (i - cnt) * 64 + 63 : (j / XRW) * 64 + j % XRW;
+            if (qon[u]) rows.load_vs(rowi, hc * ihs + igx + ue * Sact * 64, dd[u]);
+            return;
+        }
         const size_t row = qvl[u] ? ((size_t)ue * Sact + (i - cnt)) * 64 + 63 : ((size_t)ue * Sact + j / XRW) * 64 + j % XRW;
         if (qon[u]) rows.load(hb + gx + row, dd[u]);
     };
@@ -1188,8 +1324,11 @@
         int nu = (srcsh[tu] >> 18) & 0xff;
         nu = t < P ? nu : 0;
         udv[0] = wv < nu; udv[1] = wv + ne < nu;
-        udn[0] = ubase[(size_t)tu * Sact * XUCAP + (udv[0] ? wv : 0)];
-        udn[1] = ubase[(size_t)tu * Sact * XUCAP + (udv[1] ? wv + ne : 0)];
+        if constexpr (XB) { udn[0] = unit_ld(tu, udv[0] ? wv : 0); udn[1] = unit_ld(tu, udv[1] ? wv + ne : 0); }
+        else {
+            udn[0] = ubase[(size_t)tu * Sact * XUCAP + (udv[0] ? wv : 0)];
+            udn[1] = ubase[(size_t)tu * Sact * XUCAP + (udv[1] ? wv + ne : 0)];
+        }
     };
     auto take_units = [&]() {
         ud[0] = udv[0] ? make_int2(__builtin_amdgcn_readfirstlane(udn[0].x), __builtin_amdgcn_readfirstlane(udn[0].y)) : make_int2(0, 0);
@@ -1268,8 +1407,8 @@
             if constexpr (RECL) {
                 if (need0 && lane < Sact) v0 = rows.load_one(hb + gx + ((size_t)e * Sact + lane) * 64 + 63, IV);
             }
-            load_state(I0, hb, ud[0], 0);
-            load_state(I1, hb, ud[1], 0);
+            load_state(I0, hb, cur, ud[0], 0);
+            load_state(I1, hb, cur, ud[1], 0);
 #ifdef HANK_DEV_NOATOMIC
 #define lds_add(p, v) (*(p) = (v))
 #endif
@@ -1352,7 +1491,7 @@
                 const int tot = ((d.x >> 16) & 0xfff) + ((d.y >> 16) & 0xff);
                 for (int i0 = u2 < 2 * ne ? 64 : 0; i0 < tot; i0 += 64) {
                     load_rec(I0, t, d, i0);
-                    load_state(I0, hb, d, i0);
+                    load_state(I0, hb, cur, d, i0);
                     process(I0, d);
                 }
             }
@@ -1384,7 +1523,8 @@
                 double sv[SP];
 #pragma unroll
                 for (int k = 0; k < SP; k++) sv[k] = k < NSL ? mx[k] : 0.0;
-                rows.store((size_t)nxt * hs + slot, sv);
+                if constexpr (XB) rows.store_vs(lane, nxt * ihs + igx + islot, sv);
+                else rows.store((size_t)nxt * hs + slot, sv);
             }
             double at[NAP];
 #pragma unroll
@@ -1398,8 +1538,10 @@
             }
             if constexpr (VAL) {
                 if (recD) {
-                    if (own) R.Dseq[(size_t)(t + 1) * G + pt] = mx[IV];
-                    else if (virt) A.Dvirt[((size_t)t * ne + e) * 64 + cW] = mx[IV];
+                    if (own) {
+                        if constexpr (XB) buf_st64<BUF_AUX_REC>(mx[IV], rrec, ipt * 8, (int)(A.ro.Dseq + (unsigned)((t + 1) * G) * 8u));
+                        else R.Dseq[(size_t)(t + 1) * G + pt] = mx[IV];
+                    } else if (virt) A.Dvirt[((size_t)t * ne + e) * 64 + cW] = mx[IV];
                     at[IV] = live ? polr * mx[IV] : 0.0;
                     at[NSL + IV] = live ? xar * mx[IV] : 0.0;
                 }
```

Result: faster. 8516 JVPs/s (median of 6 runs) (+5.4%).
